# justinhj/minbpe-cc

Hardware: AMD Instinct MI355X
Metric: bpe_train_merges_per_sec (higher is better)
Workload: dtype u16; 1 GPU; BASELINE config 4: SplitMix64(seed 42) uniform-random bytes, 4294967296 bytes whole job, basic encoder (one chunk), vocab 32000, lexicographic tie-break; a step is ONE WHOLE TRAINING (pair-count scan, stream and table setup, every merge up to the vocabulary: 31744 merges); corpus_bytes=4294967296, vocab_size=32000

## Files before the change

### include/mbpe.h

```cpp
#ifndef MBPE_H
#define MBPE_H

#include <stdint.h>

#ifdef __cplusplus
extern "C" {
#endif

#define MBPE_API __attribute__((visibility("default")))

#define MBPE_MAX_VOCAB_BASIC   65534u
#define MBPE_MAX_VOCAB_ENDBIT  32766u
#define MBPE_MAX_VOCAB_CHUNKED 65518u
#define MBPE_MAX_VOCAB_WIDE    16777216u
#define MBPE_NO_BARRIER 0xFFFFFFFFu

typedef enum {
    MBPE_NEED_EXCHANGE =  1,
    MBPE_OK            =  0,
    MBPE_ERR_ARG       = -1,
    MBPE_ERR_NO_DEVICE = -2,
    MBPE_ERR_HIP       = -3,
    MBPE_ERR_VOCAB     = -4,
    MBPE_ERR_STATE     = -5,
    MBPE_ERR_OOM       = -6,
    MBPE_ERR_REGEX     = -7,
    MBPE_ERR_SPLIT_GAP = -8,
    MBPE_ERR_COMM      = -9,
    MBPE_ERR_OVERFLOW  = -10,
    MBPE_ERR_IO        = -11
} mbpe_status;

typedef struct mbpe_ctx mbpe_ctx;

typedef struct {
    uint64_t n_bytes;
    uint64_t n_chunks;
    uint64_t n_slots;
    uint64_t n_live;
    uint32_t n_merges;
    uint32_t n_compactions;
    uint64_t n_pairs;
    float    ms_pair_count;
    float    ms_begin;
    float    ms_steps;
    uint32_t pair_count_launches;
    uint32_t merge_launches;
    float    ms_merge_kernel;
    uint32_t n_batches;
    uint32_t n_fused;
    uint32_t n_fused_dropped;
    uint32_t cut_conflict;
    uint32_t cut_bucket;
    uint32_t cut_single;
    uint32_t cut_full;
    uint32_t n_validation_drops;
    float    ms_grow_table;
    float    ms_compact;
    uint32_t n_table_grows;
    uint32_t n_sel_fallback;
    uint32_t fused_launches;
    float    ms_fused_kernel;
    uint64_t fused_slots;
    uint32_t n_sel_retry;
    uint32_t adapt_limit;
    uint64_t n_sel_blocks;
    uint32_t size_hist[8];
    uint32_t n_skipped;
    uint32_t n_skip_cut;
    uint64_t exchange_words;
    uint32_t exchanges;
    uint32_t pad_;
    uint64_t fused_live_tokens;
    float    ms_pair_count_kernel;
    uint32_t pad2_;
} mbpe_stats;

MBPE_API const char *mbpe_last_error(void);
MBPE_API const char *mbpe_version(void);


MBPE_API int  mbpe_create(int device_id, mbpe_ctx **out);
MBPE_API void mbpe_destroy(mbpe_ctx *ctx);


MBPE_API int mbpe_load_corpus(mbpe_ctx *ctx, const uint8_t *text, uint64_t n_bytes,
                              const uint64_t *chunk_off, uint64_t n_chunks,
                              int text_on_device);

MBPE_API int mbpe_load_corpus_ranges(mbpe_ctx *ctx, const uint8_t *text, uint64_t n_bytes,
                                     const uint64_t *starts, const uint64_t *ends, uint64_t n_chunks,
                                     int text_on_device);

MBPE_API int mbpe_pair_count_u8(mbpe_ctx *ctx, uint32_t *table65536_out);


MBPE_API int mbpe_train_begin(mbpe_ctx *ctx, uint32_t vocab_size);

MBPE_API int mbpe_train_steps(mbpe_ctx *ctx, uint32_t n_steps, uint32_t *steps_done_out);

MBPE_API int mbpe_train_sequences(mbpe_ctx *ctx, uint32_t n_sequences, uint32_t *merges_done_out);

MBPE_API int mbpe_train_result(mbpe_ctx *ctx, uint32_t *merges_out, int32_t *counts_out,
                               uint32_t cap_merges, uint32_t *n_merges_out);

MBPE_API int mbpe_train_lexical(mbpe_ctx *ctx, const uint8_t *text, uint64_t n_bytes,
                                const uint64_t *chunk_off, uint64_t n_chunks,
                                uint32_t vocab_size,
                                uint32_t *merges_out, int32_t *counts_out,
                                uint32_t *n_merges_out, mbpe_stats *stats_out);

MBPE_API int mbpe_train(mbpe_ctx *ctx, const uint8_t *text, uint64_t n_bytes,
                        const uint64_t *chunk_off, uint64_t n_chunks, uint32_t vocab_size,
                        int conflict_resolution,
                        uint32_t *merges_out, int32_t *counts_out,
                        uint32_t *n_merges_out, mbpe_stats *stats_out);

MBPE_API int mbpe_get_stats(mbpe_ctx *ctx, mbpe_stats *out);


MBPE_API int mbpe_get_stream(mbpe_ctx *ctx, uint32_t *tokens_out, uint8_t *chunk_end_out,
                             uint64_t cap, uint64_t *n_out);

MBPE_API int mbpe_stream_device(mbpe_ctx *ctx, const void **slots_out, uint64_t *n_slots_out,
                                uint32_t *slot_bits_out, uint32_t *end_bit_out, uint32_t *barrier_out);

MBPE_API int mbpe_table_device(mbpe_ctx *ctx, const void **cells_out, uint32_t *vshift_out);

MBPE_API int mbpe_get_pairs(mbpe_ctx *ctx, uint32_t *first_out, uint32_t *second_out,
                            int32_t *count_out, uint64_t cap, uint64_t *n_out);

MBPE_API int mbpe_compact(mbpe_ctx *ctx);

MBPE_API int mbpe_set_option(mbpe_ctx *ctx, const char *name, int64_t value);


MBPE_API int mbpe_encode_chunks(int device_id, const uint8_t *text, uint64_t n_bytes,
                                const uint64_t *chunk_off, uint64_t n_chunks,
                                const uint32_t *merges, uint32_t n_merges,
                                uint32_t *tokens_out, uint64_t cap, uint64_t *n_out,
                                uint32_t *n_passes_out);

MBPE_API int mbpe_encode_chunks_device(int device_id, const uint8_t *text, uint64_t n_bytes,
                                       const uint64_t *chunk_off, uint64_t n_chunks,
                                       const uint32_t *merges, uint32_t n_merges,
                                       uint32_t *tokens_dev_out, uint64_t cap, uint64_t *n_out,
                                       uint32_t *n_passes_out);

typedef struct mbpe_encoder mbpe_encoder;
MBPE_API int  mbpe_encoder_create(int device_id, const uint32_t *merges, uint32_t n_merges, mbpe_encoder **out);
MBPE_API void mbpe_encoder_destroy(mbpe_encoder *e);

MBPE_API int  mbpe_encoder_encode(mbpe_encoder *e, const uint8_t *text, uint64_t n_bytes, int text_on_device,
                                  const uint64_t *chunk_off, uint64_t n_chunks,
                                  void *tokens_out, uint64_t cap, uint32_t token_bits, int out_on_device,
                                  uint64_t *chunk_tok_off_out, uint64_t *n_out, uint32_t *n_passes_out);

MBPE_API int  mbpe_encoder_set_option(mbpe_encoder *e, const char *name, int64_t value);
// ... 96 lines not shown
```

### minbpe-cc_amd/csrc/kernels.hip

```cpp
#include "mbpe_dev.h"
#include <hip/hip_ext.h>

#include <cstdlib>

namespace mbpe {

namespace {

constexpr int kWave = 64;
constexpr uint32_t kSent = 0x10000u;

__device__ __forceinline__ uint32_t lane_id() { return threadIdx.x & (kWave - 1); }
__device__ __forceinline__ uint32_t rfl(uint32_t v) { return __builtin_amdgcn_readfirstlane(v); }

typedef unsigned int u32x4 __attribute__((ext_vector_type(4)));

__device__ __forceinline__ uint32_t wave_from_next(uint32_t v, uint32_t edge) {
    return (uint32_t)__builtin_amdgcn_update_dpp((int)edge, (int)v, 0x130, 0xf, 0xf, false);
}
__device__ __forceinline__ uint32_t wave_from_prev(uint32_t v, uint32_t edge) {
    return (uint32_t)__builtin_amdgcn_update_dpp((int)edge, (int)v, 0x138, 0xf, 0xf, false);
}

#define MBPE_GLOBAL_AS __attribute__((address_space(1)))
// ... 1560 lines not shown
}

__global__ void k_apply(PairTable t, DevCtl *ctl, const unsigned long long *__restrict__ best_ptr,
                        uint32_t X, uint32_t *LR, const uint32_t *gm_gadj, TileSum *sums,
                        const TileSum *side, uint32_t *chg, uint32_t n_chg_words, int seq) {
    if (seq) {
        if (ctl->batch_n != 1) return;
        const uint32_t k = ctl->k_done;
        best_ptr += k;
        X = 256u + k;
    }
    const unsigned long long best = *best_ptr;
    const uint32_t x = blockIdx.x * blockDim.x + threadIdx.x;
    if ((best >> 32) != 0) {
        const uint32_t key = ~(uint32_t)best;
        const uint32_t a = key >> 16, b = key & 0xFFFFu;
        patch_sums(sums, side, chg, n_chg_words, x, gridDim.x * blockDim.x);
        const uint32_t pitch = lr_pitch(X);
        for (uint32_t xx = x; xx < X; xx += gridDim.x * blockDim.x) {
            const uint2 lr = make_uint2(LR[lr_idx(pitch, xx, 0, 0)], LR[lr_idx(pitch, xx, 0, 1)]);
            if (lr.x) {
                table_add(t, ctl, (xx << 16) | a, -(int32_t)lr.x, false);
                table_add(t, ctl, (xx << 16) | X, (int32_t)lr.x, true);
            }
            if (lr.y) {
                table_add(t, ctl, (b << 16) | xx, -(int32_t)lr.y, false);
                table_add(t, ctl, (X << 16) | xx, (int32_t)lr.y, true);
            }
            if (lr.x) LR[lr_idx(pitch, xx, 0, 0)] = 0;
            if (lr.y) LR[lr_idx(pitch, xx, 0, 1)] = 0;
        }
        if (x == 0) {
            const uint32_t m = gm_gadj ? gm_gadj[0] : ctl->m;
            const uint32_t adj = gm_gadj ? gm_gadj[1] : ctl->adj;
            if (m) table_add(t, ctl, (a << 16) | b, -(int32_t)m, false);
            if (adj) {
                table_add(t, ctl, (b << 16) | a, -(int32_t)adj, false);
                table_add(t, ctl, (X << 16) | X, (int32_t)adj, true);
            }
            const uint32_t rm = ctl->rm;
            ctl->removed_total += rm;
            ctl->n_live -= rm;
            ctl->m = 0;
            ctl->adj = 0;
            ctl->rm = 0;
        }
    }
}


#ifndef MBPE_PRED_NUM
#define MBPE_PRED_NUM 4
#endif
constexpr uint32_t kBucketKeys = 2;
#ifndef MBPE_LUT_BUCKETS
#define MBPE_LUT_BUCKETS 8192
#endif
constexpr uint32_t kBuckets = MBPE_LUT_BUCKETS;
static_assert((kBuckets & (kBuckets - 1u)) == 0, "the hash is masked");
constexpr uint32_t kEmptyPair = 0xFFFEFFFEu;

static_assert(kBatchMax <= 65536, "batch indices are stored in 16 bits");
constexpr uint32_t kByteCols = 256u + (uint32_t)kTTMax + 1u;
constexpr uint32_t kByteRows = 257u;
struct BatchLutHash {
    uint2 bucket[kBuckets];
    uint32_t bidx[kBuckets];
};
struct BatchLutMem : BatchLutHash {
    uint16_t byte_tail[kByteRows * kByteCols > sizeof(BatchLutHash) / 2 ? kByteRows * kByteCols - sizeof(BatchLutHash) / 2 : 1];
    __device__ __forceinline__ uint16_t *byte_tab() { return reinterpret_cast<uint16_t *>(this); }
};
static_assert(sizeof(BatchLutMem) >= kByteRows * kByteCols * 2, "the byte table overlays the hash table");
#ifndef MBPE_HASH_SEEDS
#define MBPE_HASH_SEEDS 8
#endif
constexpr int kHashSeeds = MBPE_HASH_SEEDS;
__device__ __constant__ const uint32_t kHashMul[8] = {2531u, 40503u, 10007u, 60493u, 25013u, 7919u, 52361u, 33391u};
static_assert(kHashSeeds >= 1 && kHashSeeds <= 8, "kHashMul");
struct BatchLut {
    BatchLutMem *m;
    uint32_t mul;
    bool bytes;
    uint32_t idmask;
    __device__ __forceinline__ BatchLut(BatchLutMem *mem, const BatchState *bs, uint32_t idmask_)
        : m(mem), mul(rfl(bs->hash_mul)), bytes(rfl(bs->byte_lut) != 0u), idmask(idmask_) {}
};

template <bool TT>
__device__ __forceinline__ uint32_t byte_entry(const BatchLut &lut, uint32_t first, uint32_t second, uint32_t idmask) {
    const uint32_t r = first < 256u ? first : 256u;
    uint32_t c = second < 256u ? second : kByteCols - 1u;
    if (TT) {
        const uint32_t i = idmask - 1u - second;
        c = i < (uint32_t)kTTMax ? 256u + i : c;
    }
    return lut.m->byte_tab()[r * kByteCols + c];
}

__device__ __forceinline__ uint32_t pair_hash(uint32_t mul, uint32_t first, uint32_t second) {
    return (__umul24(second, mul) + first) & (kBuckets - 1u);
}
__device__ __forceinline__ uint32_t pair_hash_u(uint32_t uniform_mul, uint32_t first, uint32_t second) {
    uint32_t h;
    asm("v_mad_u32_u24 %0, %1, %2, %3" : "=v"(h) : "v"(second), "s"(uniform_mul), "v"(first));
    return h & (kBuckets - 1u);
}

struct TTInfo {
    uint32_t map[kTTSlots];
    uint32_t tok[kTTMax];
    uint32_t pair[kTTMax];
    uint32_t cnt[kTTMax];
};

__device__ __forceinline__ void tt_build(TTInfo &ti, const BatchState *bs, uint32_t n_keys, uint32_t fake) {
    for (uint32_t i = threadIdx.x; i < kTTSlots; i += blockDim.x) ti.map[i] = 0xFFFFFFFFu;
    for (uint32_t i = threadIdx.x; i < (uint32_t)kTTMax; i += blockDim.x) { ti.tok[i] = kHole; ti.pair[i] = 0; ti.cnt[i] = 0; }
    __syncthreads();
    if (threadIdx.x == 0) {
        uint32_t n = 0;
        for (uint32_t j = 0; j < n_keys && n < (uint32_t)kTTMax; ++j) {
            const uint32_t key = bs->key[j];
            const uint32_t a = key >> 16;
            if ((key & 0xFFFFu) != a) continue;
            ti.map[a & (kTTSlots - 1u)] = a | ((fake - n) << 16);
            ti.tok[n] = a;
            ti.pair[n] = j;
            ++n;
        }
    }
    __syncthreads();
}

__device__ __forceinline__ void tt_flush(TTInfo &ti, uint32_t *hdr_m) {
    __syncthreads();
    if (threadIdx.x < (uint32_t)kTTMax && ti.cnt[threadIdx.x]) atomicAdd(&hdr_m[ti.pair[threadIdx.x]], ti.cnt[threadIdx.x]);
}

constexpr uint32_t kTTMark = 0xFFFEu;
__device__ __forceinline__ void lut_build(BatchLut &lut, const BatchState *bs, uint32_t n_keys, uint32_t fake,
                                          bool tt_marks = false) {
    if (lut.bytes) {
        uint32_t *tw = reinterpret_cast<uint32_t *>(lut.m->byte_tab());
        for (uint32_t i = threadIdx.x; i < (kByteRows * kByteCols + 1u) / 2u; i += blockDim.x) tw[i] = 0xFFFFFFFFu;
        __syncthreads();
        uint16_t *tab = lut.m->byte_tab();
        for (uint32_t j = threadIdx.x; j < n_keys; j += blockDim.x) {
            const uint32_t key = bs->key[j];
            const uint32_t a = key >> 16, b = key & 0xFFFFu;
            if (a != b) tab[a * kByteCols + b] = (uint16_t)j;
        }
        if (threadIdx.x == 0 && bs->tt_index != kNoTT) {
            uint32_t n_tt = 0;
            for (uint32_t j = bs->tt_index; j < n_keys && n_tt < (uint32_t)kTTMax; ++j) {
                const uint32_t key = bs->key[j];
                if ((key >> 16) == (key & 0xFFFFu)) {
                    tab[(key >> 16) * kByteCols + 256u + n_tt++] = (uint16_t)j;
                    if (tt_marks) tab[(key >> 16) * kByteCols + (key >> 16)] = (uint16_t)kTTMark;
                }
            }
        }
        __syncthreads();
        return;
    }
    uint32_t *words = reinterpret_cast<uint32_t *>(lut.m->bucket);
// ... 559 lines not shown
    for (int j = 0; j < 8; ++j) {
        if (s[j] != kHole) {
            if (last == kHole) first_id = s[j] & idmask;
            if ((s[j] & idmask) == last) { ++len; repeats = true; }
            else { full = full && last == kHole; len = 1; }
            lodd |= (len & 1u) ? 0u : 1u << j;
            lead |= full ? 1u << j : 0u;
            last = s[j];
        }
    }
    const bool p1_runs = h.p1 != kHole && !(h.p1 & endbit);
    const uint32_t in_last = h.p1, in_len = p1_runs ? (rb_small & 1u) : 1u;
    uint32_t rl, rn;
    const bool cross = first_id == wave_from_prev(last, in_last);
    if (__ballot(last == kHole) == 0ull && __ballot(repeats || cross) == 0ull) {
        rl = rlane(last, kWave - 1);
        rn = 1u;
    } else {
    auto join = [&](uint32_t o_last, uint32_t o_len, bool o_full) {
        if (last == kHole) { last = o_last; len = o_len; full = o_full; }
        else if (o_last != kHole) {
            if (full && (last & idmask) == o_last) { len += o_len; full = o_full; }
            else full = false;
        }
    };
    if (__ballot(last == kHole || (full && cross)) != 0ull) {
        if (lane == 0) join(in_last, in_len, false);
#pragma unroll
        for (int d = 1; d < kWave; d <<= 1) {
            const uint32_t ol = __shfl_up(last, d, kWave), on = __shfl_up(len | (full ? 0x80000000u : 0u), d, kWave);
            if (lane >= (uint32_t)d) join(ol, on & 0x7FFFFFFFu, (on >> 31) != 0u);
        }
    }
    const uint32_t lv = wave_from_prev(last, in_last), ln = wave_from_prev(len, in_len);
    const uint32_t odd = lodd ^ ((first_id == lv && (ln & 1u)) ? lead : 0u);
    if (__ballot(odd != 0u) != 0ull) {
#pragma unroll
        for (int j = 0; j < 8; ++j)
            if ((odd >> j) & 1u) s[j] = stand_in(s[j]);
    }
    rl = rlane(last, kWave - 1);
    rn = rlane(len, kWave - 1);
    }
    if (h.n1 != kHole) {
        const uint32_t n1 = h.n1;
        const bool c1 = (n1 & idmask) == rl;
        if (c1 && (rn & 1u)) h.n1 = stand_in(n1);
        rn = c1 ? rn + 1u : 1u;
        rl = n1;
        if (h.n2 != kHole && (h.n2 & idmask) == rl && (rn & 1u)) h.n2 = stand_in(h.n2);
    }
    if (p1_runs) {
        const uint32_t p1 = h.p1, p2 = h.p2;
        if (!(rb_small & 1u)) h.p1 = stand_in(p1);
        if (p2 == p1 && (rb_small & 1u)) h.p2 = stand_in(p2);
    }
}

template <int MODE>
__device__ __forceinline__ bool tt_needed(const uint32_t s[8], const uint32_t nxt[8], const Halo &h,
                                          uint32_t tile_first, const TTInfo &ti, uint32_t live_mask = 0xFFu) {
    constexpr uint32_t idmask = MODE == 1 ? 0x7FFFu : 0xFFFFu;
    auto member = [&](uint32_t v) -> bool {
        const uint32_t id = v & idmask;
        return (ti.map[id & (kTTSlots - 1u)] & 0xFFFFu) == id;
    };
    uint32_t eqm = 0;
#pragma unroll
    for (int j = 0; j < 8; ++j) eqm |= (((s[j] ^ nxt[j]) & idmask) == 0u ? 1u : 0u) << j;
    eqm &= live_mask;
    bool need = false;
    if (__ballot(eqm != 0u) != 0ull) {
#pragma unroll
        for (int j = 0; j < 8; ++j)
            if ((eqm >> j) & 1u) need = need || member(s[j]);
    }
    bool hneed = false;
    if (h.p1 != kHole && (((h.p1 ^ tile_first) & idmask) == 0u || (h.p2 != kHole && ((h.p2 ^ h.p1) & idmask) == 0u)))
        hneed = member(h.p1);
    if (h.n1 != kHole && h.n2 != kHole && ((h.n1 ^ h.n2) & idmask) == 0u) hneed = hneed || member(h.n1);
    return __ballot(need) != 0ull || hneed;
}

template <int MODE, int DIAG, bool WRITE, bool TT, class DC>
__device__ __forceinline__ uint4 fused_tile_pf(const uint4 q_orig, const uint32_t s[8], const Halo h,
                                               uint32_t old_x, uint32_t old_y, uint32_t old_z, const BatchLut &lut,
                                               uint32_t X0, uint32_t tile, TileSum *sout, uint32_t *hdr_adj, uint32_t *LR,
                                               DC &dc, bool dc_on, uint32_t &wave_rm, bool &wrote_sum,
                                               __amdgpu_buffer_rsrc_t lr_rsrc, uint32_t adj_pitch, uint16_t *stage,
                                               uint32_t *chg, bool renamed, TTInfo *ti, bool &need_rename,
                                               __amdgpu_buffer_rsrc_t t_rsrc = __amdgpu_buffer_rsrc_t(), bool use_t = false);

template <int MODE, bool HOT, bool TT, int DIAG = 0>
__global__ __launch_bounds__(kLutThreads) void k_scan_batch(const uint16_t *tok0, const uint16_t *tok1,
                                                              const TileSum *__restrict__ sin, uint32_t n_tiles,
                                                              uint32_t *__restrict__ chg, const BatchState *bs,
                                                              uint32_t *hdr_m, uint32_t *hdr_adj, uint32_t *LR,
                                                              const DevCtl *ctl, const RankEdge *le,
                                                              const RankEdge *re,
                                                              const uint32_t *__restrict__ run_in, int hot_launched,
                                                              uint32_t *T) {
    constexpr uint32_t idmask = MODE == 1 ? 0x7FFFu : 0xFFFFu;
    __shared__ BatchLutMem lut_mem;
    const uint32_t waves_per_block = kLutThreads / kWave;
    const uint32_t n_waves = gridDim.x * waves_per_block;
    __shared__ DeltaCache dc;
    const uint32_t n_keys = ctl->batch_n;
    if (n_keys < 2 || ctl->fused) return;
    if ((bs->tt_index != kNoTT) != TT) return;
    __shared__ TTInfo ti;
    const uint16_t *tok = ctl->cur ? tok1 : tok0;
    const uint32_t ctl_k_done = rfl(ctl->k_done);
    const uint32_t adj_pitch = rfl(ctl->adj_pitch);
    if (hot_mismatch<HOT>(bs->packed[0] >> 32, ctl, hot_launched)) return;
    constexpr bool dc_on = HOT;
    if (dc_on) dc_init(dc);
    BatchLut lut(&lut_mem, bs, idmask);
    lut_build(lut, bs, n_keys, idmask - 1u);
    if (TT) tt_build(ti, bs, n_keys, idmask - 1u);
    uint32_t tile = rfl(blockIdx.x * waves_per_block + threadIdx.x / kWave);
    if (tile < n_tiles) {

    const uint32_t last_tile = n_tiles - 1;
    auto clamp_tile = [&](uint64_t t) { return (uint32_t)(t < n_tiles ? t : last_tile); };
    const __amdgpu_buffer_rsrc_t sums_rsrc =
        __builtin_amdgcn_make_buffer_rsrc(const_cast<TileSum *>(sin), 0, n_tiles * 16u, 0x00020000);
    const __amdgpu_buffer_rsrc_t lr_rsrc = __builtin_amdgcn_make_buffer_rsrc(LR, 0, 0xFFFFFFFCu, 0x00020000);
    const bool use_t = T != nullptr && !HOT && ctl->cells_on != 0u && n_keys >= ctl->cells_min;
    const __amdgpu_buffer_rsrc_t t_rsrc = __builtin_amdgcn_make_buffer_rsrc(T ? T : LR, 0, T ? 0xFFFFFFFCu : 0u, 0x00020000);
    TileIn t0 = tile_issue(tok, sums_rsrc, tile);
    TileIn t1 = tile_issue(tok, sums_rsrc, clamp_tile((uint64_t)tile + n_waves));
    bool v1 = (uint64_t)tile + n_waves < n_tiles;
    for (;;) {
        const bool v2 = (uint64_t)tile + 2ull * n_waves < n_tiles;
        TileIn t2 = tile_issue(tok, sums_rsrc, clamp_tile((uint64_t)tile + 2ull * n_waves));

        const uint32_t me_nlive = rlane(t0.smw, 6) & 0xFFFFu;
        if (me_nlive != 0) {
            uint32_t s[8];
            unpack8(t0.q, s);
            Halo h;
            const uint32_t pw1 = rlane(t0.smw, 1), pw2 = rlane(t0.smw, 2);
            const uint32_t nw0 = rlane(t0.smw, 8), nw2 = rlane(t0.smw, 10);
            const bool fast = tile > 0 && tile + 1 < n_tiles && (pw2 & 0xFFFFu) >= 2 && (nw2 & 0xFFFFu) >= 2;
            if (fast) {
                h.p1 = pw1 >> 16; h.p2 = pw1 & 0xFFFFu;
                h.n1 = nw0 & 0xFFFFu; h.n2 = nw0 >> 16;
            } else {
                h = halo_slow(sin, n_tiles, tile, le, re);
            }
            uint32_t rm_unused = 0;
            bool ws_unused = false, no_rename = false;
            if (TT) tt_rename<MODE>(s, h, ti, run_in[tile]);
            fused_tile_pf<MODE, 0, false, TT>(t0.q, s, h, rlane(t0.smw, 4), rlane(t0.smw, 5), rlane(t0.smw, 6), lut,
                                              256u + ctl_k_done, tile, nullptr, hdr_adj, LR, dc, dc_on, rm_unused, ws_unused,
                                              lr_rsrc, adj_pitch, nullptr, chg, TT, &ti, no_rename, t_rsrc, use_t);
        }
        if (!v1) break;
        tile += n_waves;
        t0 = t1; t1 = t2;
        v1 = v2;
    }
    }
    if (dc_on) dc_flush(dc, LR);
    if (TT) {
        tt_flush(ti, hdr_m);
    }
}

template <int MODE, int DIAG, bool WRITE, bool TT, class DC>
__device__ __forceinline__ uint4 fused_tile_pf(const uint4 q_orig, const uint32_t s[8], const Halo h,
                                               uint32_t old_x, uint32_t old_y, uint32_t old_z, const BatchLut &lut,
                                               uint32_t X0, uint32_t tile, TileSum *sout, uint32_t *hdr_adj, uint32_t *LR,
                                               DC &dc, bool dc_on, uint32_t &wave_rm, bool &wrote_sum,
                                               __amdgpu_buffer_rsrc_t lr_rsrc, uint32_t adj_pitch, uint16_t *stage,
                                               uint32_t *chg, bool renamed, TTInfo *ti, bool &need_rename,
                                               __amdgpu_buffer_rsrc_t t_rsrc, bool use_t) {
    constexpr uint32_t idmask = MODE == 1 ? 0x7FFFu : 0xFFFFu;
    constexpr uint32_t endbit = MODE == 1 ? kEndBit : 0u;
    constexpr uint32_t kNone = 0xFFFFu;
    const uint32_t pitch = lr_pitch(X0);
    const uint32_t xcd_off = DIAG == 6 ? (__builtin_amdgcn_s_getreg((3 << 11) | 20) & 7u) * (2u * 512u * pitch) : 0u;
    auto delta_add = [&](uint32_t idx, uint32_t delta) {
        if (dc_on) dc_add(dc, true, LR, idx, delta);
        else __builtin_amdgcn_raw_ptr_buffer_atomic_add_i32((int)delta, lr_rsrc, (idx + xcd_off) << 2, 0, 0);
    };
    uint32_t lane = lane_id();
    asm volatile("" : "+v"(lane));
    const uint32_t live = old_z & 0xFFFFu;
    if (live == 0u) return q_orig;
    uint32_t tile_first = old_x & 0xFFFFu, tile_last = old_y >> 16;
    if (TT && renamed) {
        const uint32_t li = live - 1u;
        uint32_t sl = s[0];
#pragma unroll
        for (uint32_t j = 1; j < 8; ++j) sl = (li & 7u) == j ? s[j] : sl;
        tile_first = rlane(s[0], 0);
        tile_last = rlane(sl, li >> 3);
    }
    uint32_t n[8];
#pragma unroll
    for (int j = 0; j < 7; ++j) n[j] = s[j + 1];
    n[7] = wave_from_next(s[0], h.n1);
    const uint32_t ef = lane == 0 ? h.p1 : lane == 1 ? h.p2 : lane == 2 ? tile_last : (TT && lane == 3) ? h.n1 : kHole;
    const uint32_t es = (lane == 0 ? tile_first : lane == 1 ? h.p1 : (TT && lane == 3) ? h.n2 : h.n1) & idmask;
    uint32_t idx[8], eidx;
    if (lut.bytes) {
#pragma unroll
        for (int j = 0; j < 8; ++j) idx[j] = byte_entry<TT>(lut, s[j], MODE == 1 ? n[j] & idmask : n[j], idmask);
        eidx = byte_entry<TT>(lut, ef, es, idmask);
        const uint32_t all = idx[0] & idx[1] & idx[2] & idx[3] & idx[4] & idx[5] & idx[6] & idx[7] & eidx;
        if (__ballot(all != kNone) == 0ull && DIAG != 3 && DIAG != 5) return q_orig;
        if (TT) {
            bool mark = eidx == kTTMark;
#pragma unroll
            for (int j = 0; j < 8; ++j) mark = mark || idx[j] == kTTMark;
            if (__ballot(mark) != 0ull) {
                if (!renamed) { need_rename = true; return q_orig; }
#pragma unroll
                for (int j = 0; j < 8; ++j) idx[j] = idx[j] == kTTMark ? kNone : idx[j];
                eidx = eidx == kTTMark ? kNone : eidx;
            }
            eidx = lane == 3 ? kNone : eidx;
        }
    } else {
        uint32_t Hm = 0, Wm = 0;
        {
            bool second_key;
            const bool hit = pair_hit2(lut, ef, es, second_key) && !(TT && lane == 3);
            Hm = hit ? 1u : 0u;
            Wm = second_key ? 1u : 0u;
        }
#pragma unroll
        for (int j = 7; j >= 0; --j) {
            bool second_key;
            const bool hit = pair_hit2(lut, s[j], MODE == 1 ? n[j] & idmask : n[j], second_key);
            Hm = Hm + Hm + (hit ? 1u : 0u);
            Wm = Wm + Wm + (second_key ? 1u : 0u);
        }
        if (__ballot(Hm != 0u) == 0ull && DIAG != 3 && DIAG != 5) return q_orig;
#pragma unroll
        for (int j = 0; j < 8; ++j) {
            idx[j] = kNone;
            if (__ballot(((Hm >> j) & 1u) != 0u) != 0ull) {
                const uint32_t got = lut_index_known(lut, s[j], MODE == 1 ? n[j] & idmask : n[j], ((Wm >> j) & 1u) != 0u);
                idx[j] = (Hm >> j) & 1u ? got : kNone;
            }
        }
        eidx = kNone;
        if (__ballot(((Hm >> 8) & 1u) != 0u) != 0ull) {
            const uint32_t got = lut_index_known(lut, ef, es, ((Wm >> 8) & 1u) != 0u);
            eidx = (Hm >> 8) & 1u ? got : kNone;
        }
    }
    if (DIAG == 3 || DIAG == 5) {
#pragma unroll
        for (int j = 0; j < 8; ++j) asm volatile("" :: "v"(idx[j]));
        asm volatile("" :: "v"(eidx));
        return q_orig;
    }
    const uint32_t in1 = rlane(eidx, 0), in2 = rlane(eidx, 1), out1 = rlane(eidx, 2);
    {
        const uint32_t li = live - 1u;
        const bool mine = lane == (li >> 3);
#pragma unroll
        for (uint32_t j = 0; j < 8; ++j)
            if ((li & 7u) == j) { n[j] = mine ? h.n1 : n[j]; idx[j] = mine ? out1 : idx[j]; }
    }
    const uint32_t prev7 = wave_from_prev(idx[7] | (s[7] << 16), in1 | (h.p1 << 16));
    const uint32_t prev6 = wave_from_prev(idx[6], in2);
    const int lrem = (int)live - (int)(lane * 8u);
    const uint32_t Lm = lrem >= 8 ? 0xFFu : lrem <= 0 ? 0u : (1u << lrem) - 1u;
    uint32_t Am = 0, Bm = 0;
#pragma unroll
    for (int j = 0; j < 8; ++j) {
        const uint32_t pj = j == 0 ? (prev7 & 0xFFFFu) : idx[j - 1];
        Am |= (idx[j] != kNone ? 1u : 0u) << j;
        Bm |= (pj != kNone ? 1u : 0u) << j;
    }
    Bm &= Lm;
    const uint32_t ABm = Am | Bm;
    if (__ballot(ABm != 0u) == 0ull) return q_orig;

    uint32_t n2_7 = wave_from_next(n[0], h.n2);
    uint32_t n2_patch = kSent;
    if (out1 != kNone) {
        const uint32_t li = live - 1u;
        if (lane == (li >> 3)) n2_patch = li & 7u;
    }
    uint32_t out[8];
#pragma unroll
    for (int j = 0; j < 8; ++j) {
        const uint32_t self = s[j];
        uint32_t nv = ((Bm >> j) & 1u) ? kHole : self;
        if (__ballot(((Am >> j) & 1u) != 0u) != 0ull) {
            if ((Am >> j) & 1u) {
                const uint32_t p1 = j == 0 ? prev7 >> 16 : s[j > 0 ? j - 1 : 0];
                const uint32_t ppj = j == 0 ? prev6 : j == 1 ? (prev7 & 0xFFFFu) : idx[j > 1 ? j - 2 : 0];
                const uint32_t ja = idx[j];
                const uint32_t btok = n[j];
                uint32_t n2 = j < 7 ? n[j < 7 ? j + 1 : 7] : n2_7;
                n2 = n2_patch == (uint32_t)j ? h.n2 : n2;
                nv = (X0 + ja) | (btok & endbit);
                if (TT && renamed && (btok & idmask) >= idmask - (uint32_t)kTTMax)
                    atomicAdd(&ti->cnt[idmask - 1u - (btok & idmask)], 1u);
                if (DIAG != 2) {
                    const bool lo = left_open<MODE>(p1), ro = right_open<MODE>(btok, n2);
                    const uint32_t xl = p1 & idmask, yr = n2 & idmask;
                    if (use_t && lo && ro && ppj == kNone && xl < 256u && yr < 256u) {
                        __builtin_amdgcn_raw_ptr_buffer_atomic_add_i32(1, t_rsrc, ((ja << 16) | (xl << 8) | yr) << 2, 0, 0);
                    } else {
                        if (lo) {
                            if (ppj != kNone) {
                                atomicAdd(&hdr_adj[ppj * adj_pitch + ja], 1u);
                                delta_add(lr_idx(pitch, self, ppj, 1), 0xFFFFFFFFu);
                            } else {
                                delta_add(lr_idx(pitch, xl, ja, 0u), 1u);
                            }
                        }
                        if (ro) delta_add(lr_idx(pitch, yr, ja, 1u), 1u);
                    }
                }
            }
        }
        out[j] = nv;
    }
    if (TT && renamed) {
#pragma unroll
        for (int j = 0; j < 8; ++j)
            if (out[j] != kHole && (out[j] & idmask) >= idmask - (uint32_t)kTTMax)
                out[j] = ti->tok[idmask - 1u - (out[j] & idmask)] | (out[j] & endbit);
    }
    if (!WRITE) {
        if (lane == 0) atomicOr(&chg[tile >> 5], 1u << (tile & 31u));
        return q_orig;
    }
    uint32_t n_out;
    const uint4 qc = tile_compact(out, stage, n_out);
    wave_rm += live - n_out;
    uint32_t em = lane == 0 ? 3u : 0u;
    {
        const uint32_t l1 = live - 1u, l2 = live >= 2u ? live - 2u : 0u;
        em |= lane == (l1 >> 3) ? 1u << (l1 & 7u) : 0u;
        em |= lane == (l2 >> 3) ? 1u << (l2 & 7u) : 0u;
    }
    const bool edge = __ballot((ABm & em) != 0u) != 0ull;
    uint4 ns;
    if (edge || (old_z >> 16) != 1u) {
        uint32_t c[8];
        unpack8(qc, c);
        ns = wave_summary(c);
    } else {
        ns = make_uint4(old_x, old_y, (old_z & 0xFFFF0000u) | n_out, 0u);
    }
    if (lane == 0) reinterpret_cast<uint4 *>(sout)[tile] = ns;
    wrote_sum = true;
    return qc;
}

#ifndef MBPE_SKIP_PENALTY0
#define MBPE_SKIP_PENALTY0 2
#endif
#ifndef MBPE_SKIP_PENALTY_MAX
#define MBPE_SKIP_PENALTY_MAX 256
#endif
#ifndef MBPE_FUSED_WAVES
#define MBPE_FUSED_WAVES 4
#endif
template <int MODE, bool HOT, bool TT, int DIAG = 0>
__global__ __launch_bounds__(kLutThreads, MBPE_FUSED_WAVES * 256 / kLutThreads) void k_fused_batch(uint16_t *tok0, uint16_t *tok1,
                                                               const TileSum *__restrict__ sin,
                                                               TileSum *__restrict__ sout, uint32_t n_tiles,
                                                               uint32_t *__restrict__ chg, const BatchState *bs,
                                                               uint32_t *hdr_adj, uint32_t *LR, DevCtl *ctl,
                                                               const RankEdge *le, const RankEdge *re,
                                                               uint32_t *hdr_m, const uint32_t *__restrict__ run_in,
                                                               int hot_launched, uint32_t *T) {
    constexpr uint32_t idmask = MODE == 1 ? 0x7FFFu : 0xFFFFu;
    __shared__ BatchLutMem lut_mem;
    const uint32_t lane = lane_id();
    const uint32_t waves_per_block = kLutThreads / kWave;
    const uint32_t n_waves = gridDim.x * waves_per_block;
    __shared__ DeltaCacheSmall dc;
    const uint32_t n_keys = ctl->batch_n;
    if (n_keys < 2 || !ctl->fused) return;
    if ((bs->tt_index != kNoTT) != TT) return;
    __shared__ TTInfo ti;
    __shared__ __attribute__((aligned(16))) uint16_t stage_mem[kLutThreads / kWave][kTileSlots];
    uint16_t *stage = stage_mem[threadIdx.x / kWave];
    const uint16_t *tok = ctl->cur ? tok1 : tok0;
    uint16_t *dst = ctl->cur ? tok0 : tok1;
    const uint32_t X0 = 256u + ctl->k_done;
    if (hot_mismatch<HOT>(bs->packed[0] >> 32, ctl, hot_launched)) return;
    constexpr bool dc_on = HOT;
    if (dc_on) dc_init(dc);
    BatchLut lut(&lut_mem, bs, idmask);
    lut_build(lut, bs, n_keys, idmask - 1u, TT);
    if (TT) tt_build(ti, bs, n_keys, idmask - 1u);
    if (blockIdx.x == 0 && threadIdx.x == 0) ctl->marks_all = 1;
    uint32_t tile = rfl(blockIdx.x * waves_per_block + threadIdx.x / kWave);
    uint32_t wave_rm = 0;
    if (tile < n_tiles) {

    const uint32_t last_tile = n_tiles - 1;
    auto clamp_tile = [&](uint64_t t) { return (uint32_t)(t < n_tiles ? t : last_tile); };
    const __amdgpu_buffer_rsrc_t sums_rsrc =
        __builtin_amdgcn_make_buffer_rsrc(const_cast<TileSum *>(sin), 0, n_tiles * 16u, 0x00020000);
    const __amdgpu_buffer_rsrc_t lr_rsrc = __builtin_amdgcn_make_buffer_rsrc(LR, 0, 0xFFFFFFFCu, 0x00020000);
    const bool use_t = T != nullptr && !HOT && ctl->cells_on != 0u && n_keys >= ctl->cells_min;
    const __amdgpu_buffer_rsrc_t t_rsrc = __builtin_amdgcn_make_buffer_rsrc(T ? T : LR, 0, T ? 0xFFFFFFFCu : 0u, 0x00020000);
    const uint32_t adj_pitch = rfl(ctl->adj_pitch);
#ifndef MBPE_FUSED_DEPTH
#define MBPE_FUSED_DEPTH 2
#endif
    constexpr int kDepth = MBPE_FUSED_DEPTH;
    TileIn ring[kDepth];
#pragma unroll
    for (int d = 0; d < kDepth; ++d) ring[d] = tile_issue(tok, sums_rsrc, clamp_tile((uint64_t)tile + (uint64_t)d * n_waves));
    for (;;) {
        const bool v1 = (uint64_t)tile + n_waves < n_tiles;
        const TileIn t_new = tile_issue(tok, sums_rsrc, clamp_tile((uint64_t)tile + (uint64_t)kDepth * n_waves));
        const TileIn t0 = ring[0];

        uint4 outq = t0.q;
        bool wrote_sum = false;
        const uint32_t old_x = rlane(t0.smw, 4), old_y = rlane(t0.smw, 5), old_z = rlane(t0.smw, 6);
        if (DIAG == 4) {
            asm volatile("" :: "v"(t0.smw));
        } else if ((old_z & 0xFFFFu) != 0) {
            uint32_t s[8];
            unpack8(t0.q, s);
            Halo h;
            const uint32_t pw1 = rlane(t0.smw, 1), pw2 = rlane(t0.smw, 2);
            const uint32_t nw0 = rlane(t0.smw, 8), nw2 = rlane(t0.smw, 10);
            const bool fast = tile > 0 && tile + 1 < n_tiles && (pw2 & 0xFFFFu) >= 2 && (nw2 & 0xFFFFu) >= 2;
            if (fast) {
                h.p1 = pw1 >> 16; h.p2 = pw1 & 0xFFFFu;
                h.n1 = nw0 & 0xFFFFu; h.n2 = nw0 >> 16;
            } else {
                h = halo_slow(sin, n_tiles, tile, le, re);
            }
            bool renamed = false;
            bool need_rename = false;
            if (TT && !lut.bytes) {
                uint32_t nx[8];
#pragma unroll
                for (int j = 0; j < 7; ++j) nx[j] = s[j + 1];
                nx[7] = wave_from_next(s[0], h.n1);
                const uint32_t li = (old_z & 0xFFFFu) - 1u;
                const bool mine = lane == (li >> 3);
#pragma unroll
                for (uint32_t j = 0; j < 8; ++j)
                    if ((li & 7u) == j) nx[j] = mine ? h.n1 : nx[j];
                const int lrem = (int)(old_z & 0xFFFFu) - (int)(lane * 8u);
                const uint32_t lm = lrem >= 8 ? 0xFFu : lrem <= 0 ? 0u : (1u << lrem) - 1u;
                if (tt_needed<MODE>(s, nx, h, old_x & 0xFFFFu, ti, lm)) {
                    tt_rename<MODE>(s, h, ti, run_in[tile]);
                    renamed = true;
                }
            }
            outq = fused_tile_pf<MODE, DIAG, true, TT>(t0.q, s, h, old_x, old_y, old_z, lut, X0, tile, sout, hdr_adj, LR, dc,
                                                       dc_on, wave_rm, wrote_sum, lr_rsrc, adj_pitch, stage, chg, renamed, &ti,
                                                       need_rename, t_rsrc, use_t);
            if (TT && need_rename) {
                tt_rename<MODE>(s, h, ti, run_in[tile]);
                outq = fused_tile_pf<MODE, DIAG, true, TT>(t0.q, s, h, old_x, old_y, old_z, lut, X0, tile, sout, hdr_adj, LR,
                                                           dc, dc_on, wave_rm, wrote_sum, lr_rsrc, adj_pitch, stage, chg, true,
                                                           &ti, need_rename, t_rsrc, use_t);
            }
        }
        if (!wrote_sum && lane == 0) reinterpret_cast<uint4 *>(sout)[tile] = make_uint4(old_x, old_y, old_z, 0u);
        MBPE_GLOBAL_AS char *obase =
            (MBPE_GLOBAL_AS char *)uniform_ptr(reinterpret_cast<uintptr_t>(dst) + (uint64_t)tile * (kWave * 16u));
        u32x4 oq; oq.x = outq.x; oq.y = outq.y; oq.z = outq.z; oq.w = outq.w;
        __builtin_nontemporal_store(oq, (MBPE_GLOBAL_AS u32x4 *)(obase + lane * 16u));

        if (!v1) break;
        tile += n_waves;
#pragma unroll
        for (int d = 0; d + 1 < kDepth; ++d) ring[d] = ring[d + 1];
        ring[kDepth - 1] = t_new;
    }
    }
    if (dc_on) dc_flush(dc, LR);
    if (lane == 0 && wave_rm) atomicAdd(&ctl->rm, wave_rm);
    if (TT) {
        tt_flush(ti, hdr_m);
    }
}

__global__ __launch_bounds__(256) void k_pair_cells_fold(uint32_t *__restrict__ T, uint32_t *__restrict__ LR, const DevCtl *ctl) {
    __shared__ uint32_t rows[256];
    const uint32_t n = ctl->batch_n;
    if (n < ctl->cells_min || !ctl->cells_on) return;
    const uint32_t pitch = lr_pitch(256u + ctl->k_done);
    uint32_t hits = 0;
    const uint32_t t = threadIdx.x;
    for (uint32_t j = blockIdx.x; j < n; j += gridDim.x) {
        uint32_t *tj = T + (size_t)j * 65536u;
        rows[t] = 0;
        __syncthreads();
        uint32_t col = 0;
#pragma unroll 8
        for (uint32_t x = 0; x < 256u; ++x) {
            const uint32_t v = tj[x * 256u + t];
            if (__ballot(v != 0u) == 0ull) continue;
            if (v) tj[x * 256u + t] = 0;
            col += v;
            const uint32_t rs = wave_sum(v);
            if (lane_id() == 0 && rs) atomicAdd(&rows[x], rs);
        }
        __syncthreads();
        if (col) LR[lr_idx(pitch, t, j, 1u)] += col;
        if (rows[t]) LR[lr_idx(pitch, t, j, 0u)] += rows[t];
        hits += col;
        __syncthreads();
    }
    hits = wave_sum(hits);
    if (lane_id() == 0 && hits) atomicAdd(const_cast<uint32_t *>(&ctl->cell_hits), hits);
}


__global__ __launch_bounds__(kWave) void k_adj_sums(const uint32_t *__restrict__ hdr_adj, BatchState *bs, const DevCtl *ctl) {
    const uint32_t n = ctl->batch_n;
    if (n < 2) return;
    for (uint32_t j = blockIdx.x; j < n; j += gridDim.x) {
        uint32_t in = 0, out = 0;
        for (uint32_t p = threadIdx.x; p < n; p += kWave) { in += hdr_adj[p * ctl->adj_pitch + j]; out += hdr_adj[j * ctl->adj_pitch + p]; }
        in = wave_sum(in);
        out = wave_sum(out);
        if (threadIdx.x == 0) { bs->adj_in[j] = in; bs->adj_out[j] = out; }
    }
}

constexpr uint32_t kLrChunk = 4096;
__global__ __launch_bounds__(256) void k_delta_max(const uint32_t *__restrict__ LR, BatchState *bs, const DevCtl *ctl) {
    const uint32_t n_keys = ctl->batch_n;
    if (n_keys < 2) return;
    const uint32_t X = 256u + ctl->k_done;
    const uint32_t pitch = lr_pitch(X);
    const uint32_t chunks = (X + kLrChunk - 1u) / kLrChunk;
    const uint32_t n_items = 2u * n_keys * chunks;
    for (uint32_t item = blockIdx.x; item < n_items; item += gridDim.x) {
        const uint32_t row = item / chunks, x0 = (item - row * chunks) * kLrChunk;
        const uint32_t j = row >> 1, side = row & 1u, Xj = X + j;
        const uint32_t add = side ? bs->adj_out[j] : bs->adj_in[j];
        const uint32_t *cells = LR + (size_t)row * pitch;
        unsigned long long mp = 0;
#pragma unroll 4
        for (uint32_t x = x0 + threadIdx.x; x < x0 + kLrChunk && x < X; x += 256u) {
            const uint32_t v = cells[x];
            if (v) {
                const unsigned long long p = pack_best((int32_t)(v + add), side ? (Xj << 16) | x : (x << 16) | Xj);
                mp = p > mp ? p : mp;
            }
        }
        mp = wave_max_u64(mp);
        if (lane_id() == 0 && mp > __hip_atomic_load(&bs->maxp[j], __ATOMIC_RELAXED, __HIP_MEMORY_SCOPE_AGENT))
            atomicMax(&bs->maxp[j], mp);
    }
}

constexpr int kValThreads = kBatchMax < 256 ? 256 : kBatchMax > 1024 ? 1024 : kBatchMax;
constexpr int kValSlots = kBatchMax < 256 ? 256 : kBatchMax;
__global__ __launch_bounds__(256) void k_adj_max(const uint32_t *__restrict__ hdr_adj, BatchState *bs, const DevCtl *ctl) {
    const uint32_t n = ctl->batch_n;
    if (n < 2) return;
    const uint32_t X0 = 256u + ctl->k_done;
    const uint32_t n_waves = gridDim.x * (blockDim.x / kWave);
    for (uint32_t p = blockIdx.x * (blockDim.x / kWave) + threadIdx.x / kWave; p < n; p += n_waves) {
        for (uint32_t q = lane_id(); q < n; q += kWave) {
// ... 330 lines not shown
}

__global__ void k_list_marked(const uint32_t *__restrict__ chg, uint32_t n_words, uint32_t *__restrict__ list,
                              DevCtl *ctl, uint32_t n_tiles) {
    if (ctl->batch_n < 2 || (ctl->fused && ctl->commit_n == ctl->batch_n)) return;
    const uint32_t w = blockIdx.x * blockDim.x + threadIdx.x;
    uint32_t bits = w < n_words ? chg[w] : 0u;
    if (ctl->marks_all && w < n_words) {
        const uint32_t left = n_tiles - w * 32u;
        bits = left >= 32u ? 0xFFFFFFFFu : (1u << left) - 1u;
    }
    const uint32_t cnt = __popc(bits);
    const uint32_t incl = wave_incl_scan(cnt);
    const uint32_t total = __shfl(incl, kWave - 1, kWave);
    uint32_t base = 0;
    if (lane_id() == 0 && total) base = atomicAdd(&ctl->n_marked, total);
    base = __shfl(base, 0, kWave) + incl - cnt;
    while (bits) {
        list[base++] = w * 32u + (uint32_t)__builtin_ctz(bits);
        bits &= bits - 1;
    }
}

template <int MODE, bool TT>
__global__ __launch_bounds__(kLutThreads) void k_rewrite_marked(uint16_t *tok0, uint16_t *tok1,
                                                                  const TileSum *__restrict__ sin,
                                                                  TileSum *__restrict__ sout, uint32_t n_tiles,
                                                                  uint32_t *__restrict__ chg,
                                                                  const uint32_t *__restrict__ list,
                                                                  const BatchState *bs, DevCtl *ctl,
                                                                  const RankEdge *le, const RankEdge *re,
                                                                  const uint32_t *__restrict__ run_in) {
    constexpr uint32_t idmask = MODE == 1 ? 0x7FFFu : 0xFFFFu;
    __shared__ BatchLutMem lut_mem;
    if (ctl->batch_n < 2 || (ctl->fused && ctl->commit_n == ctl->batch_n)) return;
    uint16_t *tok = ctl->cur ? tok1 : tok0;
    const uint32_t n_keys = ctl->commit_n;
    if ((bs->tt_index < n_keys) != TT) return;
    __shared__ TTInfo ti;
    __shared__ __attribute__((aligned(16))) uint16_t stage_mem[kLutThreads / kWave][kTileSlots];
    uint16_t *stage = stage_mem[threadIdx.x / kWave];
    const uint32_t X0 = 256u + ctl->k_done;
    const uint32_t n_list = ctl->n_marked;
    const bool marks_all = ctl->marks_all != 0u;
    BatchLut lut(&lut_mem, bs, idmask);
    lut_build(lut, bs, n_keys, idmask - 1u);
    if (TT) tt_build(ti, bs, n_keys, idmask - 1u);
    const uint32_t lane = lane_id();
    const uint32_t waves_per_block = kLutThreads / kWave;
    const uint32_t n_waves = gridDim.x * waves_per_block;
    uint32_t i = rfl(blockIdx.x * waves_per_block + threadIdx.x / kWave);
    if (i >= n_list) return;
    const __amdgpu_buffer_rsrc_t sums_rsrc =
        __builtin_amdgcn_make_buffer_rsrc(const_cast<TileSum *>(sin), 0, n_tiles * 16u, 0x00020000);
    const uint32_t last = n_list - 1;
    auto tile_at = [&](uint64_t k) { return list[k < n_list ? k : last]; };
    uint32_t tile0 = tile_at(i), tile1 = tile_at((uint64_t)i + n_waves), tile2 = tile_at((uint64_t)i + 2ull * n_waves);
    TileIn t0 = tile_issue(tok, sums_rsrc, tile0);
    TileIn t1 = tile_issue(tok, sums_rsrc, tile1);
    uint32_t wave_rm = 0;
    for (;;) {
        const bool has_next = (uint64_t)i + n_waves < n_list;
        const uint32_t tile3 = tile_at((uint64_t)i + 3ull * n_waves);
        const TileIn t2 = tile_issue(tok, sums_rsrc, tile2);

        const uint32_t tile = tile0;
        uint32_t s[8];
        unpack8(t0.q, s);
        Halo h;
        const uint32_t pw1 = rlane(t0.smw, 1), pw2 = rlane(t0.smw, 2);
        const uint32_t nw0 = rlane(t0.smw, 8), nw2 = rlane(t0.smw, 10);
        const bool fast = tile > 0 && tile + 1 < n_tiles && (pw2 & 0xFFFFu) >= 2 && (nw2 & 0xFFFFu) >= 2;
        if (fast) {
            h.p1 = pw1 >> 16; h.p2 = pw1 & 0xFFFFu;
            h.n1 = nw0 & 0xFFFFu; h.n2 = nw0 >> 16;
        } else {
            h = halo_slow(sin, n_tiles, tile, le, re);
        }
        uint32_t rm = 0;
        bool wrote = false;
        bool no_rename = false;
        DeltaCacheSmall no_dc;
        if (TT) tt_rename<MODE>(s, h, ti, run_in[tile]);
        const uint4 qn = fused_tile_pf<MODE, 2, true, TT>(t0.q, s, h, rlane(t0.smw, 4), rlane(t0.smw, 5), rlane(t0.smw, 6), lut,
                                                          X0, tile, sout, nullptr, nullptr, no_dc, false, rm, wrote,
                                                          __amdgpu_buffer_rsrc_t(), 0u, stage, chg, TT, &ti, no_rename);
        if (wrote) {
            reinterpret_cast<uint4 *>(tok)[(uint64_t)tile * kWave + lane] = qn;
            if (lane == 0 && marks_all) atomicOr(&chg[tile >> 5], 1u << (tile & 31u));
        } else if (lane == 0 && !marks_all) {
            atomicAnd(&chg[tile >> 5], ~(1u << (tile & 31u)));
        }
        wave_rm += rm;

        if (!has_next) break;
        i += n_waves;
        tile0 = tile1; tile1 = tile2; tile2 = tile3;
        t0 = t1; t1 = t2;
    }
    if (lane == 0 && wave_rm) atomicAdd(&ctl->rm, wave_rm);
}

__global__ void k_seq_finish(DevCtl *ctl, uint32_t *fused_flag, const BatchState *bs) {
    if (blockIdx.x || threadIdx.x) return;
    const uint32_t bs_skip_n = bs->skip_n;
    const uint32_t rm_seq = ctl->batch_n >= 2 ? ctl->rm : 0u;
    if (fused_flag) *fused_flag = ctl->fused && ctl->batch_n >= 2 ? 1u : 0u;
    if (ctl->batch_n >= 2) {
        const uint32_t rm = ctl->rm;
        ctl->removed_total += rm;
        ctl->n_live -= rm;
        ctl->rm = 0;
    }
    if (ctl->batch_n >= 2) {
        uint32_t lim = ctl->adapt_limit ? ctl->adapt_limit : (uint32_t)kBatchMax;
        if (ctl->commit_n < ctl->batch_n) lim = ctl->commit_n * 2u < 4u ? 4u : ctl->commit_n * 2u;
        else if (ctl->batch_n >= lim) lim = lim * 2u;
        ctl->adapt_limit = lim > (uint32_t)kBatchMax ? (uint32_t)kBatchMax : lim;
    }
    if (ctl->skip_off) ctl->skip_off -= 1;
    if (ctl->batch_n >= 2 && ctl->skip_failed) {
        const uint32_t pen = ctl->skip_penalty ? (ctl->skip_penalty * 2u > (uint32_t)MBPE_SKIP_PENALTY_MAX ? (uint32_t)MBPE_SKIP_PENALTY_MAX : ctl->skip_penalty * 2u)
                                               : (uint32_t)MBPE_SKIP_PENALTY0;
        ctl->skip_penalty = pen;
        ctl->skip_off = pen;
    } else if (ctl->batch_n >= 2 && bs_skip_n > 0 && ctl->skip_penalty) {
        ctl->skip_penalty /= 2u;
    }
    ctl->skip_failed = 0;
    if (ctl->cells_on && ctl->cells_min >= kCellsMinBatch && ctl->batch_n >= ctl->cells_min &&
        ctl->cell_hits * 2ull < (unsigned long long)rm_seq)
        ctl->cells_on = 0;
    ctl->cell_hits = 0;
    if (ctl->fused && ctl->batch_n >= 2) {
        ctl->n_fused += 1;
        if (ctl->commit_n == ctl->batch_n) ctl->cur ^= 1u;
        else ctl->n_fused_dropped += 1;
    }
    ctl->fused = 0;
    ctl->marks_all = 0;
    if (ctl->commit_n) ctl->size_hist[31 - __builtin_clz(ctl->commit_n) > 7 ? 7 : 31 - __builtin_clz(ctl->commit_n)] += 1;
    if (fused_flag) {
        fused_flag[1] = (uint32_t)ctl->n_live;
        fused_flag[2] = (uint32_t)(ctl->n_live >> 32);
        fused_flag[3] = ctl->commit_n;
    }
    ctl->k_done += ctl->commit_n;
    ctl->batch_n = 0;
    ctl->commit_n = 0;
    ctl->n_marked = 0;
}


constexpr int kScanThreads = 256;
constexpr int kScanPerThread = 16;
constexpr uint32_t kScanChunk = kScanThreads * kScanPerThread;

__device__ __forceinline__ unsigned long long block_sum_u64(unsigned long long v, unsigned long long *sh) {
#pragma unroll
    for (int d = kWave / 2; d > 0; d >>= 1) v += shfl_xor_u64(v, d);
    __syncthreads();
    if (lane_id() == 0) sh[threadIdx.x / kWave] = v;
    __syncthreads();
    unsigned long long r = 0;
    for (uint32_t w = 0; w < blockDim.x / kWave; ++w) r += sh[w];
    return r;
}

__global__ __launch_bounds__(kScanThreads) void k_tile_scan_partial(const TileSum *__restrict__ sums,
                                                                    uint32_t n_tiles,
                                                                    unsigned long long *__restrict__ part) {
    __shared__ unsigned long long sh[kScanThreads / kWave];
    const uint64_t base = (uint64_t)blockIdx.x * kScanChunk;
    unsigned long long s = 0;
    for (uint32_t i = threadIdx.x; i < kScanChunk; i += kScanThreads)
        if (base + i < n_tiles) s += sums[base + i].n_live;
    s = block_sum_u64(s, sh);
    if (threadIdx.x == 0) part[blockIdx.x] = s;
}

__global__ __launch_bounds__(1024) void k_tile_scan_top(unsigned long long *__restrict__ part, uint32_t n_parts,
                                                        DevCtl *ctl) {
    __shared__ unsigned long long tot[1024];
    const uint32_t per = (n_parts + 1023u) / 1024u;
    const uint32_t lo = threadIdx.x * per < n_parts ? threadIdx.x * per : n_parts;
    const uint32_t hi = lo + per < n_parts ? lo + per : n_parts;
    unsigned long long s = 0;
    for (uint32_t i = lo; i < hi; ++i) s += part[i];
    tot[threadIdx.x] = s;
    __syncthreads();
    if (threadIdx.x == 0) {
        unsigned long long run = 0;
        for (int i = 0; i < 1024; ++i) { const unsigned long long v = tot[i]; tot[i] = run; run += v; }
        ctl->scan_total = run;
    }
    __syncthreads();
    unsigned long long run = tot[threadIdx.x];
    for (uint32_t i = lo; i < hi; ++i) { const unsigned long long v = part[i]; part[i] = run; run += v; }
}

__global__ __launch_bounds__(kScanThreads) void k_tile_scan_final(const TileSum *__restrict__ sums, uint32_t n_tiles,
                                                                  const unsigned long long *__restrict__ part,
                                                                  unsigned long long *__restrict__ offsets) {
    __shared__ unsigned long long th[kScanThreads];
    const uint64_t first = (uint64_t)blockIdx.x * kScanChunk + (uint64_t)threadIdx.x * kScanPerThread;
    uint32_t v[kScanPerThread];
    unsigned long long s = 0;
#pragma unroll
    for (int i = 0; i < kScanPerThread; ++i) {
        v[i] = first + i < n_tiles ? sums[first + i].n_live : 0u;
        s += v[i];
    }
    th[threadIdx.x] = s;
    __syncthreads();
    if (threadIdx.x == 0) {
        unsigned long long run = part[blockIdx.x];
// ... 304 lines not shown
    if (!v.n_tiles) return;
    const uint32_t n_chunks = (v.n_tiles + kRunChunk - 1) / kRunChunk;
    hipLaunchKernelGGL(k_run_partial, dim3(n_chunks), dim3(kRunThreads), 0, v.stream, v.sums, v.n_tiles, best, v.ctl, seq, bs,
                       v.run_part);
    hipLaunchKernelGGL(k_run_final, dim3(n_chunks), dim3(kRunThreads), 0, v.stream, v.sums, v.n_tiles, best, v.ctl, seq, bs,
                       v.run_part, v.left_edge, v.run_in);
}

void launch_merge(const StreamView &v, const BatchView &b, const unsigned long long *best, uint32_t new_id,
                  uint32_t *m_adj, int seq, const Inst &w) {
    if (!v.n_tiles) return;
    const BatchState *bs = seq ? b.bs : nullptr;
    if (inst_may_tt(w)) launch_run_lengths(v, bs, best, seq);
    static const int occ[3] = {resident_blocks(k_merge<0, false, 0>), resident_blocks(k_merge<1, false, 0>),
                               resident_blocks(k_merge<2, false, 0>)};
    const dim3 grid(tile_grid(v.n_tiles, v.n_cus, occ[slot_mode(v.endbit)])), block(kMergeThreads);
    const int hot_launched = w.hot;
#define MBPE_MERGE_ARGS v.tok, v.tok_other, v.sums, v.side, v.n_tiles, v.chg, best, new_id, b.LR, v.ctl, m_adj, v.left_edge, \
                        v.right_edge, seq, v.run_in, hot_launched
#ifdef MBPE_DIAG
    static const int diag = getenv("MBPE_MERGE_DIAG") ? atoi(getenv("MBPE_MERGE_DIAG")) : 0;
    if (diag == 1 && !v.endbit) {
        hipLaunchKernelGGL((k_merge<0, false, 1>), grid, block, 0, v.stream, MBPE_MERGE_ARGS);
        return;
    }
    if (diag == 2 && !v.endbit) {
        hipLaunchKernelGGL((k_merge<0, false, 2>), grid, block, 0, v.stream, MBPE_MERGE_ARGS);
        return;
    }
#endif
    MBPE_BY_MODE(v.endbit, {
        if (inst_takes(w, w.tt, false)) hipLaunchKernelGGL((k_merge<M, false, 0>), grid, block, 0, v.stream, MBPE_MERGE_ARGS);
        if (inst_takes(w, w.tt, true)) hipLaunchKernelGGL((k_merge<M, true, 0>), grid, block, 0, v.stream, MBPE_MERGE_ARGS);
    });
#undef MBPE_MERGE_ARGS
}

void launch_apply(const StreamView &v, const BatchView &b, PairTable t, const unsigned long long *best, uint32_t new_id,
                  const uint32_t *gm_gadj, int seq) {
    const uint32_t n_words = (v.n_tiles + 31u) / 32u;
    uint32_t blocks = (new_id + 255) / 256;
    const uint32_t want = (n_words + 255) / 256;
    if (want > blocks) blocks = want < 2048 ? want : 2048;
    hipLaunchKernelGGL(k_apply, dim3(blocks), dim3(256), 0, v.stream, t, v.ctl, best, new_id, b.LR, gm_gadj, v.sums, v.side,
                       v.chg, n_words, seq);
}

void launch_patch_sums(const StreamView &v, const unsigned long long *best, int seq) {
    const uint32_t n_words = (v.n_tiles + 31u) / 32u;
    uint32_t blocks = (n_words + 255) / 256;
    if (blocks > 2048) blocks = 2048;
    if (blocks < 1) blocks = 1;
    hipLaunchKernelGGL(k_patch_sums, dim3(blocks), dim3(256), 0, v.stream, best, v.sums, v.side, v.chg, n_words, v.ctl, seq,
                       v.n_tiles);
}

void launch_select_batch(const StreamView &v, const BatchView &b, PairTable t, unsigned long long *best,
                         const SelectArgs &a, int attempts, int first_attempt, bool fallback) {
    const hipStream_t s = v.stream;
    const uint32_t fake_id = (v.endbit == kEndBit ? 0x7FFFu : 0xFFFFu) - 1u;
    const uint32_t tt_max = 256u + a.n_target <= fake_id + 1u - (uint32_t)kTTMax ? (uint32_t)kTTMax : 1u;
    const uint32_t sel_cap = a.sel_cap < 64u ? 64u : a.sel_cap > kSelCap ? kSelCap : a.sel_cap;
    if (a.sel) {
        const int blocks = (v.n_cus > 0 ? v.n_cus : 256) * 4;
        for (int attempt = first_attempt < 0 ? 0 : first_attempt; attempt < (attempts < 1 ? 1 : attempts > 3 ? 3 : attempts); ++attempt) {
            hipLaunchKernelGGL(k_sel_scan, dim3(blocks), dim3(256), 0, s, t, v.ctl, a.sel, a.n_target, sel_cap, attempt);
            hipLaunchKernelGGL(k_sel_pick, dim3(1), dim3(kPickThreads), 0, s, v.ctl, b.bs, a.sel, best, a.n_target, a.max_batch,
                               a.fused_min, (uint32_t)v.n_ranks, attempt, fake_id, sel_cap, tt_max, a.byte_table ? 1u : 0u);
        }
    }
    if (fallback)
        hipLaunchKernelGGL(k_select_batch, dim3(1), dim3(kHierThreads), 0, s, t, v.ctl, b.bs, best, a.n_target, a.max_batch,
                           a.fused_min, (uint32_t)v.n_ranks);
}

void launch_fused_batch(const StreamView &v, const BatchView &b, const Inst &w) {
    if (!v.n_tiles) return;
    static const int occ[3] = {resident_blocks(k_fused_batch<0, false, false, 0>, kLutThreads),
                               resident_blocks(k_fused_batch<1, false, false, 0>, kLutThreads),
                               resident_blocks(k_fused_batch<2, false, false, 0>, kLutThreads)};
    const dim3 grid(tile_grid(v.n_tiles, v.n_cus, occ[slot_mode(v.endbit)], kLutThreads)), block(kLutThreads);
    const int hot_launched = w.hot;
#define MBPE_FUSED_ARGS v.tok, v.tok_other, v.sums, v.side, v.n_tiles, v.chg, b.bs, b.hdr_adj, b.LR, v.ctl, v.left_edge, \
                        v.right_edge, b.hdr_m, v.run_in, hot_launched, b.pair_cells
#ifdef MBPE_DIAG
    const int diag = getenv("MBPE_FUSED_DIAG") ? atoi(getenv("MBPE_FUSED_DIAG")) : 0;
#define MBPE_FUSED_DIAG_CASE(D)                                                                                            \
    if (diag == D && !v.endbit) {                                                                                          \
        hipLaunchKernelGGL((k_fused_batch<0, false, false, D>), grid, block, 0, v.stream, MBPE_FUSED_ARGS);                \
        hipLaunchKernelGGL((k_fused_batch<0, false, true, D>), grid, block, 0, v.stream, MBPE_FUSED_ARGS);                 \
        return;                                                                                                            \
    }
    MBPE_FUSED_DIAG_CASE(2)
    MBPE_FUSED_DIAG_CASE(3)
    MBPE_FUSED_DIAG_CASE(4)
    MBPE_FUSED_DIAG_CASE(5)
    MBPE_FUSED_DIAG_CASE(6)
#undef MBPE_FUSED_DIAG_CASE
#endif
    MBPE_BY_MODE(v.endbit, MBPE_BY_INST(w, hipLaunchKernelGGL((k_fused_batch<M, HOT, TT>), grid, block, 0, v.stream, MBPE_FUSED_ARGS)));
#undef MBPE_FUSED_ARGS
}

void launch_scan_batch(const StreamView &v, const BatchView &b, const Inst &w) {
    if (!v.n_tiles) return;
    static const int occ[3] = {resident_blocks(k_scan_batch<0, false, false, 0>, kLutThreads),
                               resident_blocks(k_scan_batch<1, false, false, 0>, kLutThreads),
                               resident_blocks(k_scan_batch<2, false, false, 0>, kLutThreads)};
    const dim3 grid(tile_grid(v.n_tiles, v.n_cus, occ[slot_mode(v.endbit)], kLutThreads)), block(kLutThreads);
    const int hot_launched = w.hot;
    MBPE_BY_MODE(v.endbit, MBPE_BY_INST(w, hipLaunchKernelGGL((k_scan_batch<M, HOT, TT, 0>), grid, block, 0, v.stream, v.tok,
                                                             v.tok_other, v.sums, v.n_tiles, v.chg, b.bs, b.hdr_m, b.hdr_adj, b.LR,
                                                             v.ctl, v.left_edge, v.right_edge, v.run_in, hot_launched,
                                                             b.pair_cells)));
}

void launch_pair_cells_fold(const StreamView &v, const BatchView &b, uint32_t n_hint) {
    if (!b.pair_cells) return;
    if (n_hint < 64u) n_hint = 64u;
    if (n_hint > 1024u) n_hint = 1024u;
    hipLaunchKernelGGL(k_pair_cells_fold, dim3(n_hint), dim3(256), 0, v.stream, b.pair_cells, b.LR, v.ctl);
}

void launch_batch_tables(const StreamView &v, const BatchView &b, PairTable t, uint32_t id_upper, uint32_t n_hint) {
    const hipStream_t s = v.stream;
    if (n_hint < 64u) n_hint = 64u;
    if (n_hint > (uint32_t)kBatchMax) n_hint = kBatchMax;
    const uint64_t cells = (uint64_t)id_upper * kBatchMax;
    uint32_t blocks = (uint32_t)((cells + 255) / 256);
    if (blocks > 2048) blocks = 2048;
    if (blocks < 8) blocks = 8;
    hipLaunchKernelGGL(k_adj_sums, dim3(n_hint), dim3(kWave), 0, s, b.hdr_adj, b.bs, v.ctl);
    hipLaunchKernelGGL(k_delta_max, dim3(blocks < 1024 ? blocks : 1024), dim3(256), 0, s, b.LR, b.bs, v.ctl);
    hipLaunchKernelGGL(k_adj_max, dim3(n_hint / 4), dim3(256), 0, s, b.hdr_adj, b.bs, v.ctl);
    hipLaunchKernelGGL(k_validate, dim3(1), dim3(kValThreads), 0, s, t, v.ctl, b.bs, b.hdr_m, b.hdr_adj, b.LR);
    if (t.cells) {
        uint32_t j_parts = (n_hint + kApplyTile - 1) / kApplyTile;
        if (j_parts > kApplyJParts) j_parts = kApplyJParts;
        uint32_t grid = ((id_upper + kApplyTile - 1) / kApplyTile) * j_parts;
        if (grid < 256u) grid = 256u;
        hipLaunchKernelGGL(k_apply_batch_dense, dim3(grid), dim3(256), 0, s, t, v.ctl, b.bs, b.hdr_m, b.hdr_adj, b.LR, j_parts);
    } else {
        hipLaunchKernelGGL(k_apply_batch, dim3(blocks), dim3(256), 0, s, t, v.ctl, b.bs, b.hdr_m, b.hdr_adj, b.LR);
    }
}

void launch_rewrite_marked(const StreamView &v, const BatchView &b, const Inst &w) {
    if (!v.n_tiles) return;
    const uint32_t n_words = (v.n_tiles + 31u) / 32u;
    hipLaunchKernelGGL(k_list_marked, dim3((n_words + 255) / 256), dim3(256), 0, v.stream, v.chg, n_words, v.tile_list, v.ctl,
                       v.n_tiles);
    static const int occ[3] = {resident_blocks(k_rewrite_marked<0, false>, kLutThreads),
                               resident_blocks(k_rewrite_marked<1, false>, kLutThreads),
                               resident_blocks(k_rewrite_marked<2, false>, kLutThreads)};
    const dim3 grid(tile_grid(v.n_tiles, v.n_cus, occ[slot_mode(v.endbit)], kLutThreads)), block(kLutThreads);
#define MBPE_REWRITE_ARGS v.tok, v.tok_other, v.sums, v.side, v.n_tiles, v.chg, v.tile_list, b.bs, v.ctl, v.left_edge, \
                          v.right_edge, v.run_in
    MBPE_BY_MODE(v.endbit, {
        hipLaunchKernelGGL((k_rewrite_marked<M, false>), grid, block, 0, v.stream, MBPE_REWRITE_ARGS);
        if (inst_may_tt(w)) hipLaunchKernelGGL((k_rewrite_marked<M, true>), grid, block, 0, v.stream, MBPE_REWRITE_ARGS);
    });
#undef MBPE_REWRITE_ARGS
}

__global__ void k_seq_info(const DevCtl *ctl, const BatchState *bs, const unsigned long long *best, uint32_t *out) {
    if (blockIdx.x || threadIdx.x) return;
    const uint32_t n = ctl->batch_n;
    unsigned long long top = 0;
    uint32_t tt = 0;
    if (n >= 2) {
        top = bs->packed[0] >> 32;
        tt = bs->tt_index != kNoTT ? 1u : 0u;
    } else if (n == 1) {
        const unsigned long long b = best[ctl->k_done];
        const uint32_t key = ~(uint32_t)b;
        top = b >> 32;
        tt = (top != 0 && (key >> 16) == (key & 0xFFFFu)) ? 1u : 0u;
    }
    out[0] = ctl->k_done;
    out[1] = n;
    out[2] = ctl->fused;
    out[3] = tt;
    out[4] = dc_wanted(top, ctl->n_live * ctl->n_ranks) ? 1u : 0u;
    out[5] = ctl->k_limit;
    out[6] = ctl->sel_ok;
    out[7] = 0;
}

void launch_seq_info(const StreamView &v, const BatchView &b, const unsigned long long *best, uint32_t *out) {
    hipLaunchKernelGGL(k_seq_info, dim3(1), dim3(64), 0, v.stream, v.ctl, b.bs, best, out);
}

void launch_seq_finish(const StreamView &v, const BatchView &b, uint32_t *fused_flag) {
    hipLaunchKernelGGL(k_seq_finish, dim3(1), dim3(64), 0, v.stream, v.ctl, fused_flag, b.bs);
}

void launch_tile_scan(const StreamView &v, unsigned long long *offsets) {
    if (!v.n_tiles) return;
    unsigned long long *part = offsets + v.n_tiles;
    const uint32_t n_parts = (v.n_tiles + kScanChunk - 1) / kScanChunk;
    hipLaunchKernelGGL(k_tile_scan_partial, dim3(n_parts), dim3(kScanThreads), 0, v.stream, v.sums, v.n_tiles, part);
    hipLaunchKernelGGL(k_tile_scan_top, dim3(1), dim3(1024), 0, v.stream, part, n_parts, v.ctl);
    hipLaunchKernelGGL(k_tile_scan_final, dim3(n_parts), dim3(kScanThreads), 0, v.stream, v.sums, v.n_tiles, part, offsets);
}

void launch_compact_scatter(const StreamView &v, const unsigned long long *offsets) {
    if (!v.n_tiles) return;
    hipLaunchKernelGGL(k_compact_scatter, dim3(tile_grid(v.n_tiles, v.n_cus)), dim3(kMergeThreads), 0, v.stream, v.tok, v.sums,
                       offsets, v.n_tiles, v.tok_other);
}

void launch_rank_edge(const StreamView &v, uint32_t *hdr) {
    hipLaunchKernelGGL(k_rank_edge, dim3(1), dim3(64), 0, v.stream, v.sums, v.n_tiles, reinterpret_cast<RankEdge *>(hdr + 2) + v.rank,
                       v.ctl, hdr);
}

void launch_compose_edges(hipStream_t s, uint32_t *hdr, int rank, int n_ranks, RankEdge *left, RankEdge *right) {
    hipLaunchKernelGGL(k_compose_edges, dim3(1), dim3(64), 0, s, hdr, rank, n_ranks, left, right);
}

void launch_boundary_pairs(hipStream_t s, uint32_t *bp, const uint32_t *hdr, int n_ranks, uint32_t endbit, uint32_t *pcount) {
    hipLaunchKernelGGL(k_boundary_pairs, dim3(1), dim3(64), 0, s, bp, hdr, n_ranks, endbit, pcount);
}

void launch_pair_total(hipStream_t s, const uint32_t *bp, const uint32_t *pcount, unsigned long long expect,
                       unsigned long long *sum_out, DevCtl *ctl) {
    hipLaunchKernelGGL(k_pair_total, dim3(1), dim3(1024), 0, s, bp, pcount, expect, sum_out, ctl);
}

}
```

### minbpe-cc_amd/csrc/mbpe_dev.h

```cpp
#ifndef MBPE_DEV_H
#define MBPE_DEV_H

#include <hip/hip_runtime.h>
#include <stdint.h>

namespace mbpe {

constexpr uint32_t kHole = 0xFFFFu;
constexpr uint32_t kEndBit = 0x8000u;
constexpr uint32_t kBarrier = 0xFFEEu;

constexpr int kTile = 512;
constexpr int kMergeThreads = 256;
#ifndef MBPE_LUT_THREADS
#define MBPE_LUT_THREADS 1024
#endif
constexpr int kLutThreads = MBPE_LUT_THREADS;
constexpr int kSlotsPerLane = 8;

struct __attribute__((aligned(16))) TileSum {
    uint16_t head0, head1;
    uint16_t tail1, tail0;
    uint16_t n_live;
    uint16_t tail_run;
    uint16_t pad0, pad1;
};
static_assert(sizeof(TileSum) == 16, "TileSum must be 16 bytes");

struct RankEdge {
    uint32_t head0, head1;
    uint32_t tail1, tail0;
    uint32_t n_live_lo, n_live_hi;
    uint32_t tail_run_lo, tail_run_hi;
};

constexpr uint32_t kEmptyKey = 0xFFFFFFFFu;
constexpr unsigned long long kEmptySlot = 0xFFFFFFFFFFFFFFFFull;

constexpr int kBlockShift = 10;
constexpr uint32_t kBlockSize = 1u << kBlockShift;

struct PairTable {
    unsigned long long *hslot;
    uint32_t *ekey;
    int32_t  *ecnt;
    unsigned long long *bmax;
    unsigned long long *smax;
    uint32_t  hmask;
    uint32_t  ecap;
    uint32_t *cells;
    uint32_t  vshift;
};
constexpr uint32_t kPresent = 0x80000000u;

struct DevCtl {
    uint32_t n_entries;
    uint32_t err;
    uint32_t m;
    uint32_t adj;
    unsigned long long removed_total;
    unsigned long long n_live;
    unsigned long long scan_total;
    uint32_t rm;
    uint32_t k_done;
    uint32_t k_limit;
    uint32_t batch_n;
    uint32_t commit_n;
    uint32_t n_batches;
    uint32_t n_marked;
    uint32_t cur;
    uint32_t fused;
    uint32_t n_fused;
    uint32_t n_fused_dropped;
    uint32_t cut_conflict, cut_bucket, cut_single, cut_full;
    uint32_t n_validation_drops;
    unsigned long long sel_T;
    uint32_t sel_n;
    uint32_t sel_ok;
    uint32_t n_sel_fallback;
    uint32_t sel_retry;
    uint32_t adapt_limit;
    uint32_t recent_n;
    uint32_t n_sel_retry;
    uint32_t sel_mode;
    uint32_t n_ranks;
    uint32_t size_hist[8];
    uint32_t n_skipped;
    uint32_t n_skip_cut;
    uint32_t skip_off;
    uint32_t skip_penalty;
    uint32_t skip_failed;
    uint32_t skip_red_q16;
    unsigned long long n_sel_blocks;
    uint32_t first_mode;
    uint32_t first_tie;
    uint32_t marks_all;
    uint32_t cells_on;
    uint32_t cell_hits;
    uint32_t cells_min;
    uint32_t adj_pitch;

};

#ifndef MBPE_BATCH_MAX
#define MBPE_BATCH_MAX 4096
#endif
constexpr int kBatchMax = MBPE_BATCH_MAX;
constexpr int kBatchDefault = kBatchMax;
static_assert((kBatchMax & (kBatchMax - 1)) == 0 && kBatchMax >= 64,
              "a power of two: grid strides over the delta arrays keep a thread on one pair index");
#ifndef MBPE_SEL_CAP
#define MBPE_SEL_CAP 8192
#endif
constexpr uint32_t kSelCap = MBPE_SEL_CAP;
struct SelList {
    unsigned long long packed[kSelCap];
    uint32_t eidx[kSelCap];
};

#ifndef MBPE_TT_MAX
#define MBPE_TT_MAX 16
#endif
constexpr int kTTMax = MBPE_TT_MAX;
static_assert(0xFFFFu - (uint32_t)MBPE_TT_MAX > kBarrier, "the barrier id must lie below the stand-in ids");
constexpr uint32_t kTTSlots = 256;
#ifndef MBPE_SKIP_MAX
#define MBPE_SKIP_MAX 32
#endif
constexpr int kSkipMax = MBPE_SKIP_MAX;
constexpr uint32_t kCellsMinBatch = 512;
constexpr uint32_t kNoTT = 0xFFFFFFFFu;
struct BatchState {
    uint32_t key[kBatchMax];
    uint32_t eidx[kBatchMax];
    unsigned long long packed[kBatchMax];
    unsigned long long maxp[kBatchMax];
    uint32_t adj_in[kBatchMax];
    uint32_t adj_out[kBatchMax];
    uint32_t tt_index;
    uint32_t tt_token;
    uint32_t tt_n;
    uint32_t hash_mul;
    uint32_t byte_lut;
    uint32_t skip_n;
    uint32_t skip_key[kSkipMax];
    uint32_t skip_pos[kSkipMax];
    unsigned long long skip_packed[kSkipMax];
};

inline uint32_t batch_header_words(uint32_t adj_pitch) { return (uint32_t)kBatchMax + adj_pitch * adj_pitch; }
__host__ __device__ inline uint32_t lr_pitch(uint32_t ids) { return (ids + 63u) & ~63u; }
__host__ __device__ inline unsigned long long lr_words(uint32_t ids, uint32_t n_pairs) {
    return 2ull * (n_pairs ? n_pairs : 1u) * lr_pitch(ids);
}

constexpr uint32_t kErrTableFull   = 1u;
constexpr uint32_t kErrNegCount    = 2u;
constexpr uint32_t kErrMissingPair = 4u;
constexpr uint32_t kErrCountRange  = 8u;
constexpr uint32_t kErrHotSkipped  = 16u;

__host__ __device__ inline unsigned long long pack_best(int32_t count, uint32_t key) {
    return ((unsigned long long)(uint32_t)count << 32) | (uint32_t)(~key);
}

struct StreamView {
    hipStream_t stream;
    uint16_t *tok, *tok_other;
    TileSum *sums;
    TileSum *side;
    uint32_t n_tiles;
    uint32_t *chg;
    uint32_t *tile_list;
    uint32_t *run_in;
    unsigned long long *run_part;
    DevCtl *ctl;
    const RankEdge *left_edge, *right_edge;
    int rank, n_ranks;
    uint32_t endbit;
    int n_cus;
};

struct BatchView {
    BatchState *bs;
    uint32_t *hdr_m, *hdr_adj;
    uint32_t *LR;
    uint32_t *pair_cells;
};

struct Inst { bool known, tt, hot; };
inline Inst inst_any(bool hot_possible) { return Inst{false, false, hot_possible}; }
inline Inst inst_known(bool tt, bool hot) { return Inst{true, tt, hot}; }
inline bool inst_takes(const Inst &w, bool tt, bool hot) { return w.known ? w.tt == tt && w.hot == hot : !hot || w.hot; }
inline bool inst_may_tt(const Inst &w) { return !w.known || w.tt; }

void launch_fill_u32(hipStream_t s, uint32_t *p, uint64_t n, uint32_t v);
void launch_fill_u16(hipStream_t s, uint16_t *p, uint64_t n, uint16_t v);

size_t pair_count_scratch_bytes(int n_workgroups);
void launch_pair_count_u8(hipStream_t s, const uint8_t *text, uint64_t n,
                          const uint8_t *endmask, uint32_t *bp, int n_workgroups, uint32_t *scratch,
                          hipEvent_t start = nullptr, hipEvent_t stop = nullptr);

void launch_widen(hipStream_t s, const uint8_t *text, uint64_t n, const uint8_t *endmask,
                  uint16_t *tok, uint64_t n_slots_padded);
void launch_widen_barrier(hipStream_t s, const uint8_t *text, uint64_t n, const uint8_t *endmask,
                          uint16_t *tok, uint64_t n_slots);

void launch_summarize(const StreamView &v);

void launch_table_init(hipStream_t s, const uint32_t *bp, PairTable t, DevCtl *ctl);
void launch_table_rehash(hipStream_t s, PairTable t, DevCtl *ctl);

void launch_argmax(hipStream_t s, PairTable t, const DevCtl *ctl, unsigned long long *best, bool hierarchical);

size_t first_state_bytes();
void launch_first_init(hipStream_t s, void *fs);
void launch_first_tiebreak(const StreamView &v, PairTable t, unsigned long long *best, void *fs, uint32_t *xf, int seq,
                           int phase);

void launch_merge(const StreamView &v, const BatchView &b, const unsigned long long *best, uint32_t new_id,
                  uint32_t *m_adj, int seq, const Inst &w);
void launch_run_lengths(const StreamView &v, const BatchState *bs, const unsigned long long *best, int seq);

void launch_apply(const StreamView &v, const BatchView &b, PairTable t, const unsigned long long *best, uint32_t new_id,
                  const uint32_t *gm_gadj, int seq);
void launch_patch_sums(const StreamView &v, const unsigned long long *best, int seq);

struct SelectArgs {
    SelList *sel;
    uint32_t n_target, max_batch, fused_min, sel_cap;
    bool byte_table;
};
void launch_select_batch(const StreamView &v, const BatchView &b, PairTable t, unsigned long long *best,
                         const SelectArgs &a, int attempts = 3,
                         int first_attempt = 0 ,
                         bool fallback = true );
void launch_scan_batch(const StreamView &v, const BatchView &b, const Inst &w);
void launch_fused_batch(const StreamView &v, const BatchView &b, const Inst &w);
void launch_pair_cells_fold(const StreamView &v, const BatchView &b, uint32_t n_hint);
void launch_batch_tables(const StreamView &v, const BatchView &b, PairTable t, uint32_t id_upper, uint32_t n_hint);
void launch_rewrite_marked(const StreamView &v, const BatchView &b, const Inst &w);
void launch_seq_info(const StreamView &v, const BatchView &b, const unsigned long long *best, uint32_t *out);
void launch_seq_finish(const StreamView &v, const BatchView &b, uint32_t *fused_flag);

inline size_t tile_scan_scratch(uint32_t n_tiles) { return (size_t)n_tiles / 4096 + 2; }
void launch_tile_scan(const StreamView &v, unsigned long long *offsets);
void launch_compact_scatter(const StreamView &v, const unsigned long long *offsets);

inline uint32_t exchange_header_words(int n_ranks) { return (uint32_t)((2 + 8 * n_ranks + 3) / 4 * 4); }
void launch_rank_edge(const StreamView &v, uint32_t *hdr);
void launch_compose_edges(hipStream_t s, uint32_t *hdr, int rank, int n_ranks, RankEdge *left, RankEdge *right);
constexpr uint32_t kPairCountWords = 4;
void launch_boundary_pairs(hipStream_t s, uint32_t *bp, const uint32_t *hdr, int n_ranks, uint32_t endbit,
                           uint32_t *pcount);
void launch_pair_total(hipStream_t s, const uint32_t *bp, const uint32_t *pcount, unsigned long long expect,
// ... 6 lines not shown
```

### minbpe-cc_amd/csrc/train.cpp

```cpp
#include "mbpe.h"
#include "mbpe_dev.h"
#include "wide.h"
#include "hip_host.h"

#include <dlfcn.h>
#include <rccl/rccl.h>

#include <algorithm>
#include <chrono>
#include <cstddef>
#include <cstdio>
#include <cstring>
#include <map>
#include <string>
#include <unordered_map>
#include <vector>

using namespace mbpe;

namespace {

#define HIPCHK(expr) MBPE_HIP_CHECK(expr, false)

uint64_t round_up(uint64_t v, uint64_t m) { return (v + m - 1) / m * m; }
// ... 7 lines not shown
bool stoi_parses(const uint8_t *s, uint64_t n) { long long v; return stoi_value(s, n, &v); }

template <typename T>
void dfree(T *&p) {
    if (p) { (void)hipFree(p); p = nullptr; }
}

}

struct mbpe_ctx;
namespace {
template <typename T> hipError_t tmalloc(mbpe_ctx *c, T **p, size_t bytes);
template <typename T> void tfree(mbpe_ctx *c, T *&p);
void pool_trim(mbpe_ctx *c);
}

namespace {
struct Rccl {
    void *lib = nullptr;
    int (*GetUniqueId)(void *) = nullptr;
    int (*CommInitRank)(void **, int, ncclUniqueId, int) = nullptr;
    int (*CommDestroy)(void *) = nullptr;
    int (*AllReduce)(const void *, void *, size_t, int, int, void *, hipStream_t) = nullptr;
    const char *(*GetErrorString)(int) = nullptr;
    bool ok = false;
    std::string why;
};

Rccl &rccl() {
    static Rccl r;
    static bool tried = false;
    if (tried) return r;
    tried = true;
    for (const char *n : {"librccl.so.1", "librccl.so", "/opt/rocm/lib/librccl.so.1"}) {
        r.lib = dlopen(n, RTLD_NOW | RTLD_LOCAL);
        if (r.lib) break;
    }
    if (!r.lib) { r.why = "librccl.so.1 not found"; return r; }
#define MBPE_BIND(field, name) \
    r.field = reinterpret_cast<decltype(r.field)>(dlsym(r.lib, name)); \
    if (!r.field) { r.why = std::string("missing RCCL symbol ") + name; return r; }
    MBPE_BIND(GetUniqueId, "ncclGetUniqueId")
    MBPE_BIND(CommInitRank, "ncclCommInitRank")
    MBPE_BIND(CommDestroy, "ncclCommDestroy")
    MBPE_BIND(AllReduce, "ncclAllReduce")
    MBPE_BIND(GetErrorString, "ncclGetErrorString")
#undef MBPE_BIND
    r.ok = true;
    return r;
}
}

struct mbpe_ctx {
    int device = 0;
    hipStream_t stream = nullptr;
    hipEvent_t ev0 = nullptr, ev1 = nullptr;
    int n_cus = 256;

    const uint8_t *d_text = nullptr;
    uint8_t *d_text_owned = nullptr;
    uint8_t *d_endmask = nullptr;
    uint64_t n_bytes = 0;
    uint64_t n_chunks = 0;
    bool chunked = false;
    uint64_t n_barriers = 0;
    bool barrier = false;
    bool loaded = false;
    bool inert = false;

    uint32_t *pc_scratch = nullptr;
    uint32_t *pc_bp = nullptr;
    void *first_state = nullptr;
    uint32_t *xf = nullptr;

    uint16_t *tok[2] = {nullptr, nullptr};
    int cur = 0;
    uint64_t cap_slots = 0;
    uint64_t n_slots = 0;
    uint32_t n_tiles = 0;
    TileSum *sums = nullptr;
    TileSum *side = nullptr;
    uint32_t *chg = nullptr;
    uint32_t *tile_list = nullptr;
    SelList *sel = nullptr;
    uint32_t *run_in = nullptr;
    int seq_slot = -1;
    unsigned long long *offsets = nullptr;

    PairTable tab = {};
    uint32_t hcap = 0;
    DevCtl *ctl = nullptr;
    unsigned long long *best = nullptr;
    uint32_t *xb = nullptr;
    uint32_t hdr_words = 0;
    uint32_t hdrb_words = 0;
    uint32_t *hdr_m = nullptr, *hdr_adj = nullptr;
    uint32_t *LR = nullptr;
    BatchState *bs = nullptr;
    uint32_t *xb0 = nullptr;
    uint32_t h_pcount[kPairCountWords] = {};
    uint32_t *pair_cells = nullptr;
    RankEdge *d_left = nullptr, *d_right = nullptr;

    uint32_t vocab_size = 0;
    uint32_t n_target = 0;
    uint32_t k = 0;
    uint32_t n_valid = 0;
    bool begun = false;
    bool exhausted = false;
    double merges_per_seq = 0;
    uint32_t first_b = 0, first_s = 0;
    bool first_legacy = false;
    DevCtl h_ctl = {};

    int rank = 0, n_ranks = 1;
    bool comm_external = false;
    void *nccl_comm = nullptr;
    int pending = 0;
    uint32_t pending_target = 0;

    int64_t opt_compact_den = 16;
    int64_t opt_batch = 16;
    int64_t opt_time_kernels = 0;
    int64_t opt_force_exchange = 0;
    int64_t opt_hier_argmax = -1;
    int64_t opt_multi_merge = 1;
    int64_t opt_max_batch = kBatchDefault;
    int64_t opt_fused_min = 24;
    bool opt_byte_table = true;
    int64_t opt_sel_cap = kSelCap;
    int64_t opt_threshold_select = 1;
    int64_t opt_dense_table = -1;
    int hot_possible = 1;
    unsigned long long last_top = ~0ull;
    int64_t opt_barrier = -1;
    int64_t opt_first_batches = 0;
    int64_t opt_first = 0;
    int64_t opt_pc_repeat = 1;
    uint32_t k_upper = 0;
    int sel_attempts = 3;
    uint32_t max_batch_eff = kBatchMax, adj_pitch = kBatchMax;
    uint32_t *h_seq = nullptr;
    uint32_t *d_seq_info = nullptr;
    int64_t opt_pair_cells = -1;
    int64_t opt_lockstep = -1;
    hipEvent_t ev_sel = nullptr;
    std::vector<hipEvent_t> kev;
    std::vector<hipEvent_t> kev_f;
    uint32_t *seq_flags = nullptr;
    std::vector<uint32_t> h_seq_flags;

    bool wide = false;
    bool wide_active = false;
    uint32_t vocab_total = 0;
    uint32_t n_target_total = 0;
    int64_t opt_wide_from = -1;
    int64_t opt_first_wide = 0;
    bool wfirst = false;
    uint32_t *wtok[2] = {nullptr, nullptr};
    int wcur = 0;
    uint32_t *wval = nullptr, *wscratch = nullptr;
    WideTable wtab = {};
    WideCtl *wctl = nullptr;
    WideBest *wbest = nullptr;
    unsigned long long *warg = nullptr;
    WideFirst *wfs = nullptr;
    uint64_t wn_upper = 0;
    uint32_t wk = 0;
    WideCtl h_wctl = {};
    std::vector<WideBest> h_wbest;

    mbpe_stats stats = {};

    std::unordered_map<void *, size_t> pool_live;
    std::multimap<size_t, void *> pool_idle;
};

namespace {

template <typename T>
hipError_t tmalloc(mbpe_ctx *c, T **p, size_t bytes) {
    if (bytes == 0) bytes = 4;
    auto it = c->pool_idle.find(bytes);
    if (it != c->pool_idle.end()) {
        *p = static_cast<T *>(it->second);
        c->pool_live[it->second] = bytes;
        c->pool_idle.erase(it);
        return hipSuccess;
    }
    void *q = nullptr;
    hipError_t e = hipMalloc(&q, bytes);
    if (e == hipErrorOutOfMemory && !c->pool_idle.empty()) {
        pool_trim(c);
        e = hipMalloc(&q, bytes);
    }
    if (e != hipSuccess) return e;
    c->pool_live[q] = bytes;
    *p = static_cast<T *>(q);
    return hipSuccess;
}

template <typename T>
void tfree(mbpe_ctx *c, T *&p) {
    if (!p) return;
    auto it = c->pool_live.find((void *)p);
    if (it != c->pool_live.end()) {
        c->pool_idle.emplace(it->second, it->first);
        c->pool_live.erase(it);
    } else {
        (void)hipFree((void *)p);
    }
    p = nullptr;
}

template <typename T>
void trelease(mbpe_ctx *c, T *p) {
    if (!p) return;
    c->pool_live.erase((void *)p);
    (void)hipFree((void *)p);
}

void pool_trim(mbpe_ctx *c) {
    for (auto &kv : c->pool_idle) (void)hipFree(kv.second);
    c->pool_idle.clear();
}

int sync_ctl(mbpe_ctx *c) {
    HIPCHK(hipMemcpyAsync(&c->h_ctl, c->ctl, sizeof(DevCtl), hipMemcpyDeviceToHost, c->stream));
    HIPCHK(hipStreamSynchronize(c->stream));
    c->cur = (int)(c->h_ctl.cur & 1u);
#ifdef MBPE_DIAG
    if (getenv("MBPE_MERGE_DIAG") || getenv("MBPE_FUSED_DIAG")) c->h_ctl.err = 0;
#endif
    if (c->h_ctl.err) {
        char buf[320];
        snprintf(buf, sizeof(buf), "device error flags 0x%x (1=pair table full, 2=negative count, 4=missing pair, "
                                   "8=a pair occurs 2^31 times or more, or the byte-pair counts do not add up to the "
                                   "pairs scanned (a count reached 2^32), 16=a stream pass was skipped)",
                 c->h_ctl.err);
        mbpe_host::set_last_error(buf);
        return MBPE_ERR_OVERFLOW;
    }
    return MBPE_OK;
}

void free_training(mbpe_ctx *c) {
    tfree(c, c->tok[0]); tfree(c, c->tok[1]);
    tfree(c, c->sums); tfree(c, c->side); tfree(c, c->chg); tfree(c, c->tile_list);
    tfree(c, c->offsets);
    tfree(c, c->tab.hslot); tfree(c, c->tab.ekey); tfree(c, c->tab.ecnt); tfree(c, c->tab.cells);
    tfree(c, c->tab.bmax); tfree(c, c->tab.smax);
    tfree(c, c->ctl); tfree(c, c->best); tfree(c, c->xb); tfree(c, c->xb0); tfree(c, c->pair_cells);
    tfree(c, c->d_left); tfree(c, c->d_right); tfree(c, c->bs); tfree(c, c->sel); tfree(c, c->seq_flags); tfree(c, c->run_in);
    tfree(c, c->first_state);
    tfree(c, c->xf);
    tfree(c, c->wtok[0]); tfree(c, c->wtok[1]); tfree(c, c->wval); tfree(c, c->wscratch);
    tfree(c, c->wtab.keys); tfree(c, c->wtab.cnts); tfree(c, c->wctl); tfree(c, c->wbest); tfree(c, c->warg);
    tfree(c, c->wfs);
    c->wtab = {};
    c->wfirst = false;
    c->wide_active = false;
    c->wk = 0;
    c->wn_upper = 0;
    c->h_wbest.clear();
    c->LR = nullptr;
    c->pending = 0;
    c->begun = false;
    c->k = c->n_valid = 0;
    c->exhausted = false;
}

void free_corpus(mbpe_ctx *c) {
    dfree(c->d_text_owned);
    dfree(c->d_endmask);
    c->d_text = nullptr;
    c->loaded = false;
}

static inline bool dense_possible(const mbpe_ctx *c) { return c->vocab_size <= 32768; }
static inline bool use_dense(const mbpe_ctx *c) {
    if (!dense_possible(c)) return false;
    if (c->wide) return false;
    return c->opt_dense_table != 0;
}

int alloc_table_dense(mbpe_ctx *c) {
    uint32_t vshift = 8;
    while ((1u << vshift) < c->vocab_size) ++vshift;
    c->tab = {};
    c->tab.vshift = vshift;
    c->tab.ecap = 1u << (2 * vshift);
    const size_t cells = (size_t)1 << (2 * vshift);
    HIPCHK(tmalloc(c, &c->tab.cells, cells * 4));
    HIPCHK(hipMemsetAsync(c->tab.cells, 0, cells * 4, c->stream));
    const size_t nb = (cells >> kBlockShift) + 2, ns = (cells >> (2 * kBlockShift)) + 2;
    HIPCHK(tmalloc(c, &c->tab.bmax, nb * 8));
    HIPCHK(tmalloc(c, &c->tab.smax, ns * 8));
    HIPCHK(hipMemsetAsync(c->tab.bmax, 0, nb * 8, c->stream));
    HIPCHK(hipMemsetAsync(c->tab.smax, 0, ns * 8, c->stream));
    return MBPE_OK;
}

int alloc_table(mbpe_ctx *c, uint32_t ecap) {
    c->tab.ecap = ecap;
    c->hcap = next_pow2((uint64_t)ecap * 2);
    c->tab.hmask = c->hcap - 1;
    HIPCHK(tmalloc(c, &c->tab.hslot, (size_t)c->hcap * 8));
    HIPCHK(tmalloc(c, &c->tab.ekey, (size_t)ecap * 4));
    HIPCHK(tmalloc(c, &c->tab.ecnt, (size_t)ecap * 4));
    const size_t nb = ((size_t)ecap >> kBlockShift) + 2, ns = ((size_t)ecap >> (2 * kBlockShift)) + 2;
    HIPCHK(tmalloc(c, &c->tab.bmax, nb * 8));
    HIPCHK(tmalloc(c, &c->tab.smax, ns * 8));
    HIPCHK(hipMemsetAsync(c->tab.bmax, 0, nb * 8, c->stream));
    HIPCHK(hipMemsetAsync(c->tab.smax, 0, ns * 8, c->stream));
    launch_fill_u32(c->stream, reinterpret_cast<uint32_t *>(c->tab.hslot), (uint64_t)c->hcap * 2, 0xFFFFFFFFu);
    return MBPE_OK;
}

uint64_t batch_headroom(const mbpe_ctx *c, uint32_t steps) {
    uint64_t per = 2ull * c->vocab_size + 1;
    return per * steps;
}

uint64_t table_cap_limit(const mbpe_ctx *c) {
    uint64_t v = c->vocab_size;
    uint64_t lim = v * v;
    if (lim > (1ull << 30)) lim = 1ull << 30;
    return std::max<uint64_t>(lim, 1024);
}

struct WallTimer {
    float *acc;
    std::chrono::steady_clock::time_point t0 = std::chrono::steady_clock::now();
    explicit WallTimer(float *a) : acc(a) {}
    ~WallTimer() { *acc += std::chrono::duration<float, std::milli>(std::chrono::steady_clock::now() - t0).count(); }
};

int grow_table(mbpe_ctx *c, uint64_t want) {
    if (c->tab.cells) return MBPE_OK;
    WallTimer timer(&c->stats.ms_grow_table);
    c->stats.n_table_grows++;
    uint64_t lim = table_cap_limit(c);
    uint64_t ecap = std::min<uint64_t>(std::max<uint64_t>(want, (uint64_t)c->tab.ecap * 4), lim);
    if (ecap <= c->tab.ecap) return MBPE_OK;
    PairTable old = c->tab;
    c->tab = {};
    int rc = alloc_table(c, (uint32_t)ecap);
    if (rc != MBPE_OK) return rc;
    uint32_t n = c->h_ctl.n_entries;
    HIPCHK(hipMemcpyAsync(c->tab.ekey, old.ekey, (size_t)n * 4, hipMemcpyDeviceToDevice, c->stream));
    HIPCHK(hipMemcpyAsync(c->tab.ecnt, old.ecnt, (size_t)n * 4, hipMemcpyDeviceToDevice, c->stream));
    HIPCHK(hipMemcpyAsync(c->tab.bmax, old.bmax, (((size_t)old.ecap >> kBlockShift) + 2) * 8,
                          hipMemcpyDeviceToDevice, c->stream));
    HIPCHK(hipMemcpyAsync(c->tab.smax, old.smax, (((size_t)old.ecap >> (2 * kBlockShift)) + 2) * 8,
                          hipMemcpyDeviceToDevice, c->stream));
    launch_table_rehash(c->stream, c->tab, c->ctl);
    HIPCHK(hipStreamSynchronize(c->stream));
    trelease(c, old.hslot); trelease(c, old.ekey); trelease(c, old.ecnt);
    trelease(c, old.bmax); trelease(c, old.smax);
    return MBPE_OK;
}

int ensure_pc_scratch(mbpe_ctx *c) {
    if (!c->pc_scratch) HIPCHK(hipMalloc(&c->pc_scratch, pair_count_scratch_bytes(c->n_cus)));
    return MBPE_OK;
}

int ensure_events(std::vector<hipEvent_t> &pool, size_t n) {
    while (pool.size() < n) {
        hipEvent_t e;
        HIPCHK(hipEventCreate(&e));
        pool.push_back(e);
    }
    return MBPE_OK;
}

inline uint32_t endbit_of(const mbpe_ctx *c) { return !c->chunked ? 0u : c->barrier ? kBarrier : kEndBit; }

inline bool is_multi(const mbpe_ctx *c) { return c->n_ranks > 1 || c->opt_force_exchange; }

enum TokOrder { kBuffers01, kLiveFirst };

StreamView stream_view(const mbpe_ctx *c, TokOrder order) {
    const int first = order == kLiveFirst ? c->cur : 0;
    const bool multi = is_multi(c);
    StreamView v = {};
    v.stream = c->stream;
    v.tok = c->tok[first], v.tok_other = c->tok[1 - first];
    v.sums = c->sums, v.side = c->side, v.n_tiles = c->n_tiles;
    v.chg = c->chg, v.tile_list = c->tile_list;
    v.run_in = c->run_in, v.run_part = c->offsets + c->n_tiles;
    v.ctl = c->ctl;
    v.left_edge = multi ? c->d_left : nullptr, v.right_edge = multi ? c->d_right : nullptr;
    v.rank = c->rank, v.n_ranks = std::max(1, c->n_ranks);
    v.endbit = endbit_of(c), v.n_cus = c->n_cus;
    return v;
}

BatchView batch_view(const mbpe_ctx *c) { return BatchView{c->bs, c->hdr_m, c->hdr_adj, c->LR, c->pair_cells}; }

int do_compact(mbpe_ctx *c) {
    if (!c->n_tiles) return MBPE_OK;
    WallTimer timer(&c->stats.ms_compact);
    const int dst = 1 - c->cur;
    const StreamView v = stream_view(c, kLiveFirst);
    launch_tile_scan(v, c->offsets);
    launch_compact_scatter(v, c->offsets);
    const uint64_t live = c->h_ctl.n_live;
    const uint64_t padded = std::max<uint64_t>(round_up(live, kTile), kTile);
    launch_fill_u16(c->stream, c->tok[dst] + live, padded - live, (uint16_t)kHole);
    c->cur = dst;
    c->n_slots = padded;
    c->n_tiles = (uint32_t)(padded / kTile);
    launch_summarize(stream_view(c, kLiveFirst));
    DevCtl patch = c->h_ctl;
    patch.removed_total = 0;
    HIPCHK(hipMemcpyAsync(&c->ctl->removed_total, &patch.removed_total, sizeof(patch.removed_total),
                          hipMemcpyHostToDevice, c->stream));
    HIPCHK(hipMemsetD32Async(reinterpret_cast<hipDeviceptr_t>(&c->ctl->cur), c->cur, 1, c->stream));
    c->h_ctl.cur = (uint32_t)c->cur;
    HIPCHK(hipStreamSynchronize(c->stream));
    c->h_ctl.removed_total = 0;
    c->stats.n_compactions++;
    return MBPE_OK;
}

}

namespace mbpe_host {
int ctx_device(const mbpe_ctx *c) { return c->device; }
}

extern "C" {

int mbpe_create(int device_id, mbpe_ctx **out) {
    if (!out) { mbpe_host::set_last_error("mbpe_create: out is NULL"); return MBPE_ERR_ARG; }
    *out = nullptr;
    int n = 0;
    hipError_t e = hipGetDeviceCount(&n);
    if (e != hipSuccess || n <= 0 || device_id < 0 || device_id >= n) {
        mbpe_host::set_last_error("no usable HIP device (the MI355X path has no CPU fallback)");
        return MBPE_ERR_NO_DEVICE;
    }
    HIPCHK(hipSetDevice(device_id));
    mbpe_ctx *c = new mbpe_ctx();
    c->device = device_id;
    hipDeviceProp_t prop;
    if (hipGetDeviceProperties(&prop, device_id) == hipSuccess) c->n_cus = prop.multiProcessorCount;
    if (hipStreamCreateWithFlags(&c->stream, hipStreamNonBlocking) != hipSuccess ||
        hipEventCreate(&c->ev0) != hipSuccess || hipEventCreate(&c->ev1) != hipSuccess ||
        hipEventCreateWithFlags(&c->ev_sel, hipEventDisableTiming) != hipSuccess ||
        hipHostMalloc(reinterpret_cast<void **>(&c->h_seq), 64, hipHostMallocDefault) != hipSuccess) {
        mbpe_host::set_last_error("could not create HIP stream / events");
        delete c;
        return MBPE_ERR_HIP;
    }
    *out = c;
    return MBPE_OK;
}

void mbpe_destroy(mbpe_ctx *c) {
    if (!c) return;
    (void)hipSetDevice(c->device);
    if (c->stream) (void)hipStreamSynchronize(c->stream);
    free_training(c);
    pool_trim(c);
    free_corpus(c);
    dfree(c->pc_scratch);
    dfree(c->pc_bp);
    if (c->nccl_comm && rccl().ok) rccl().CommDestroy(c->nccl_comm);
    for (hipEvent_t e : c->kev) (void)hipEventDestroy(e);
    for (hipEvent_t e : c->kev_f) (void)hipEventDestroy(e);
    if (c->ev0) (void)hipEventDestroy(c->ev0);
    if (c->ev1) (void)hipEventDestroy(c->ev1);
    if (c->ev_sel) (void)hipEventDestroy(c->ev_sel);
    if (c->h_seq) (void)hipHostFree(c->h_seq);
    dfree(c->d_seq_info);
    if (c->stream) (void)hipStreamDestroy(c->stream);
    delete c;
}

int mbpe_set_option(mbpe_ctx *c, const char *name, int64_t value) {
    if (!c || !name) return MBPE_ERR_ARG;
    std::string n(name);
    if (n == "compact_den") c->opt_compact_den = value;
    else if (n == "batch") c->opt_batch = std::max<int64_t>(1, value);
    else if (n == "time_kernels") c->opt_time_kernels = value;
    else if (n == "force_exchange") c->opt_force_exchange = value;
    else if (n == "hier_argmax") c->opt_hier_argmax = value;
    else if (n == "multi_merge") c->opt_multi_merge = value;
    else if (n == "max_batch") c->opt_max_batch = std::min<int64_t>(std::max<int64_t>(1, value), kBatchMax);
    else if (n == "fused_min") c->opt_fused_min = std::max<int64_t>(2, value);
    else if (n == "dense_table") c->opt_dense_table = value;
    else if (n == "threshold_select") c->opt_threshold_select = value != 0;
    else if (n == "conflict_resolution") {
        if (value != 0 && value != 1) { mbpe_host::set_last_error("conflict_resolution: 0 = first, 1 = lexical"); return MBPE_ERR_ARG; }
        if (c->begun && (c->pending || (c->k < c->n_target && !c->exhausted))) {
            mbpe_host::set_last_error("conflict_resolution cannot change in the middle of a training");
            return MBPE_ERR_STATE;
        }
        c->opt_first = value == 0;
    }
    else if (n == "chunk_barrier") c->opt_barrier = value < 0 ? -1 : value != 0;
    else if (n == "first_batches") c->opt_first_batches = value != 0;
    else if (n == "sel_cap") c->opt_sel_cap = std::min<int64_t>(std::max<int64_t>(64, value), kSelCap);
    else if (n == "byte_table") c->opt_byte_table = value != 0;
    else if (n == "lockstep") c->opt_lockstep = value < 0 ? -1 : value != 0;
    else if (n == "pair_cells") c->opt_pair_cells = value < 0 ? -1 : value != 0;
    else if (n == "wide_from") c->opt_wide_from = value < 0 ? -1 : value;
    else if (n == "first_wide") c->opt_first_wide = value != 0;
    else if (n == "pc_repeat") c->opt_pc_repeat = std::min<int64_t>(std::max<int64_t>(1, value), 1000);
    else { mbpe_host::set_last_error("unknown option " + n); return MBPE_ERR_ARG; }
    return MBPE_OK;
}

int mbpe_load_corpus(mbpe_ctx *c, const uint8_t *text, uint64_t n_bytes, const uint64_t *chunk_off,
                     uint64_t n_chunks, int text_on_device) {
    if (!c || (!text && n_bytes)) { mbpe_host::set_last_error("mbpe_load_corpus: NULL argument"); return MBPE_ERR_ARG; }
    HIPCHK(hipSetDevice(c->device));
    free_training(c);
    free_corpus(c);
    if (n_bytes != c->n_bytes || (chunk_off != nullptr) != c->chunked) pool_trim(c);
    c->n_bytes = n_bytes;
    c->chunked = chunk_off != nullptr;
    c->n_chunks = chunk_off ? n_chunks : 1;
    c->n_barriers = 0;
    c->barrier = false;
    c->inert = false;
    if (chunk_off) {
        if (chunk_off[0] != 0 || chunk_off[n_chunks] != n_bytes) {
            mbpe_host::set_last_error("chunk_off must start at 0 and end at n_bytes");
            return MBPE_ERR_ARG;
        }
        for (uint64_t i = 0; i < n_chunks; ++i)
            if (chunk_off[i] > chunk_off[i + 1]) {
                mbpe_host::set_last_error("chunk_off must be ascending");
                return MBPE_ERR_ARG;
            }
    }
    if (text_on_device && ((uintptr_t)text & 15)) {
        mbpe_host::set_last_error("device text must be 16-byte aligned");
        return MBPE_ERR_ARG;
    }

    std::vector<uint8_t> tmp;
    const uint8_t *h_text = text;
    if (text_on_device && n_bytes) {
        bool need_all = chunk_off != nullptr;
        uint64_t take = need_all ? n_bytes : std::min<uint64_t>(n_bytes, 64);
        tmp.resize(take);
        HIPCHK(hipMemcpy(tmp.data(), text, take, hipMemcpyDeviceToHost));
        h_text = tmp.data();
    }
    const uint64_t n_vec = (n_bytes + 15) / 16;
    std::vector<uint8_t> mask;
    if (chunk_off) {
        mask.assign(n_vec * 2 + 16, 0);
        uint64_t dropped = 0;
        for (uint64_t ci = 0; ci < n_chunks; ++ci) {
            uint64_t s = chunk_off[ci], e = chunk_off[ci + 1];
            if (e == s) continue;
            mask[(e - 1) >> 3] |= (uint8_t)(1u << ((e - 1) & 7));
            if (h_text[s] == 0 && stoi_parses(h_text + s + 1, e - s - 1)) {
                for (uint64_t i = s; i < e; ++i) mask[i >> 3] |= (uint8_t)(1u << (i & 7));
                dropped++;
            }
        }
        c->n_chunks = n_chunks - dropped;
        uint64_t ends = 0;
        for (uint8_t b : mask) ends += (uint64_t)__builtin_popcount(b);
        c->n_barriers = ends;
    } else if (n_bytes && h_text[0] == 0) {
        uint64_t have = text_on_device ? tmp.size() : n_bytes;
        bool parses = stoi_parses(h_text + 1, have - 1);
        if (!parses && text_on_device && have < n_bytes) {
            bool all_ws = true;
            for (uint64_t i = 1; i < have; ++i)
                if (!(h_text[i] == ' ' || (h_text[i] >= 9 && h_text[i] <= 13))) { all_ws = false; break; }
            if (all_ws) {
                tmp.resize(n_bytes);
                HIPCHK(hipMemcpy(tmp.data(), text, n_bytes, hipMemcpyDeviceToHost));
                parses = stoi_parses(tmp.data() + 1, n_bytes - 1);
            }
        }
        c->inert = parses;
        if (parses) c->n_chunks = 0;
    }

    if (text_on_device) {
        c->d_text = text;
    } else {
// ... 53 lines not shown
        w += ends[i] - starts[i];
    }
    off[n_chunks] = w;
    return mbpe_load_corpus(c, buf.data(), packed, off.data(), n_chunks, 0);
}

static uint64_t pairs_scanned(const mbpe_ctx *c) {
    if (c->chunked) return c->n_bytes - c->n_barriers;
    return c->inert || c->n_bytes < 2 ? 0 : c->n_bytes - 1;
}

int mbpe_pair_count_u8(mbpe_ctx *c, uint32_t *table65536_out) {
    if (!c) return MBPE_ERR_ARG;
    if (!c->loaded) { mbpe_host::set_last_error("mbpe_pair_count_u8: no corpus loaded"); return MBPE_ERR_STATE; }
    HIPCHK(hipSetDevice(c->device));
    int rcs = ensure_pc_scratch(c);
    if (rcs != MBPE_OK) return rcs;
    if (!c->pc_bp) HIPCHK(hipMalloc(&c->pc_bp, 65536 * 4 + 16));
    uint32_t *bp = c->pc_bp;
    HIPCHK(hipMemsetAsync(bp, 0, 65536 * 4, c->stream));
    const int reps = table65536_out ? 1 : (int)std::max<int64_t>(1, c->opt_pc_repeat);
    rcs = ensure_events(c->kev, 2ull * reps);
    if (rcs != MBPE_OK) return rcs;
    HIPCHK(hipEventRecord(c->ev0, c->stream));
    if (!c->inert)
        for (int r = 0; r < reps; ++r)
            launch_pair_count_u8(c->stream, c->d_text, c->n_bytes, c->d_endmask, bp, c->n_cus, c->pc_scratch,
                                 c->kev[2 * r], c->kev[2 * r + 1]);
    HIPCHK(hipEventRecord(c->ev1, c->stream));
    unsigned long long *sum_dev = reinterpret_cast<unsigned long long *>(bp + 65536);
    if (reps == 1) launch_pair_total(c->stream, bp, nullptr, 0, sum_dev, nullptr);
    hipError_t e = hipStreamSynchronize(c->stream);
    if (e == hipSuccess) e = hipGetLastError();
    if (e == hipSuccess && table65536_out) e = hipMemcpy(table65536_out, bp, 65536 * 4, hipMemcpyDeviceToHost);
    unsigned long long sum = 0;
    if (e == hipSuccess && reps == 1) e = hipMemcpy(&sum, sum_dev, 8, hipMemcpyDeviceToHost);
    if (e != hipSuccess) { mbpe_host::set_last_error(hip_err("pair count", e)); return MBPE_ERR_HIP; }
    if (reps == 1 && sum != pairs_scanned(c)) {
        mbpe_host::set_last_error("mbpe_pair_count_u8: the counts add up to " + std::to_string(sum) + " of " +
                                  std::to_string(pairs_scanned(c)) + " pairs: a pair occurs 2^32 times or more");
        return MBPE_ERR_OVERFLOW;
    }
    HIPCHK(hipEventElapsedTime(&c->stats.ms_pair_count, c->ev0, c->ev1));
    c->stats.ms_pair_count /= (float)reps;
    c->stats.ms_pair_count_kernel = 0;
    if (!c->inert && c->n_bytes >= 2) {
        float sum = 0;
        for (int r = 0; r < reps; ++r) {
            float km = 0;
            HIPCHK(hipEventElapsedTime(&km, c->kev[2 * r], c->kev[2 * r + 1]));
            sum += km;
        }
        c->stats.ms_pair_count_kernel = sum / (float)reps;
    }
    c->stats.pair_count_launches += (uint32_t)reps;
#ifdef MBPE_PC_STAMPS
    {
        std::vector<unsigned long long> st((size_t)c->n_cus * 16);
        HIPCHK(hipMemcpy(st.data(), reinterpret_cast<const char *>(c->pc_scratch) + (size_t)c->n_cus * 32768 * 4, st.size() * 8,
                         hipMemcpyDeviceToHost));
        unsigned long long t0 = ~0ull;
        for (int w = 0; w < c->n_cus; ++w) if (st[16 * w] && st[16 * w] < t0) t0 = st[16 * w];
        for (int k = 0; k < 16; ++k) {
            double lo = 1e30, hi = 0, sum = 0; int cnt = 0;
            for (int w = 0; w < c->n_cus; ++w) {
                if (!st[16 * w + k]) continue;
                const double us = (double)(st[16 * w + k] - t0) * 0.01;
                lo = std::min(lo, us); hi = std::max(hi, us); sum += us; ++cnt;
            }
            if (cnt) fprintf(stderr, "pc stamp %2d: min %8.2f avg %8.2f max %8.2f us (%d workgroups)\n", k, lo, sum / cnt, hi, cnt);
        }
    }
#endif
    return MBPE_OK;
}


static inline bool use_hier(const mbpe_ctx *c) {
    if (c->opt_hier_argmax >= 0) return c->opt_hier_argmax != 0;
    if (c->tab.cells) return c->tab.ecap > (1u << 20);
    return c->h_ctl.n_entries > (1u << 20);
}

static int begin_local(mbpe_ctx *c, uint32_t vocab_size) {
    free_training(c);
    c->vocab_size = vocab_size;
    c->n_target = vocab_size - 256;
    c->k = 0;
    c->n_valid = 0;
    c->exhausted = false;
    c->first_legacy = false;
    c->sel_attempts = 3;
    c->merges_per_seq = 0;
    c->first_b = c->first_s = 0;

    const uint64_t n = c->inert ? 0 : c->n_bytes;
    const uint64_t n_bar = c->barrier ? c->n_barriers : 0;
    const uint64_t dense_slots = std::max<uint64_t>(round_up(n + n_bar, kTile), kTile);
    c->n_slots = c->barrier ? std::max<uint64_t>(2 * round_up(n, kTile / 2), kTile) : dense_slots;
    c->cap_slots = dense_slots;
    if (c->n_slots / kTile > 0x0FFFFFF0ull) { mbpe_host::set_last_error("corpus shard too large"); return MBPE_ERR_ARG; }
    c->n_tiles = (uint32_t)(c->n_slots / kTile);
    c->hdr_words = exchange_header_words(c->n_ranks);
    c->max_batch_eff = (uint32_t)std::min<int64_t>(c->opt_max_batch, is_multi(c) ? 1024 : kBatchMax);
    c->adj_pitch = (uint32_t)round_up(std::max<uint32_t>(c->max_batch_eff, 64u), 64);
    c->hdrb_words = (batch_header_words(c->adj_pitch) + 3) / 4 * 4;
    HIPCHK(tmalloc(c, &c->tok[0], c->n_slots * 2));
    HIPCHK(tmalloc(c, &c->tok[1], c->cap_slots * 2));
    HIPCHK(tmalloc(c, &c->sums, (size_t)c->n_tiles * sizeof(TileSum)));
    HIPCHK(tmalloc(c, &c->side, (size_t)c->n_tiles * sizeof(TileSum)));
    HIPCHK(tmalloc(c, &c->chg, ((size_t)c->n_tiles / 32 + 2) * 4));
    HIPCHK(tmalloc(c, &c->tile_list, ((size_t)c->n_tiles + 64) * 4));
    HIPCHK(hipMemsetAsync(c->chg, 0, ((size_t)c->n_tiles / 32 + 2) * 4, c->stream));
    HIPCHK(tmalloc(c, &c->offsets, ((size_t)c->n_tiles + tile_scan_scratch(c->n_tiles)) * 8));
    const size_t xb_words = (size_t)c->hdr_words + c->hdrb_words + lr_words(vocab_size, c->max_batch_eff) + 8;
    const size_t xb0_words = 65536 + (size_t)c->hdr_words + kPairCountWords;
    HIPCHK(tmalloc(c, &c->xb, xb_words * 4));
    HIPCHK(tmalloc(c, &c->xb0, xb0_words * 4));
    HIPCHK(hipMemsetAsync(c->xb, 0, xb_words * 4, c->stream));
    HIPCHK(hipMemsetAsync(c->xb0, 0, xb0_words * 4, c->stream));
    if (c->opt_pair_cells > 0 || (c->opt_pair_cells < 0 && c->n_slots >= (64ull << 20))) {
        const size_t cells = (size_t)c->max_batch_eff * 65536u;
        HIPCHK(tmalloc(c, &c->pair_cells, cells * 4));
        HIPCHK(hipMemsetAsync(c->pair_cells, 0, cells * 4, c->stream));
    }
    c->hdr_m = c->xb + c->hdr_words;
    c->hdr_adj = c->hdr_m + kBatchMax;
    c->LR = c->xb + c->hdr_words + c->hdrb_words;
    HIPCHK(tmalloc(c, &c->bs, sizeof(BatchState)));
    HIPCHK(tmalloc(c, &c->sel, sizeof(SelList)));
    HIPCHK(tmalloc(c, &c->run_in, ((size_t)c->n_tiles + 64) * 4));
    HIPCHK(tmalloc(c, &c->seq_flags, 4096 * 4 * 4));
    HIPCHK(hipMemsetAsync(c->bs, 0, sizeof(BatchState), c->stream));
    if (c->opt_first) {
        HIPCHK(tmalloc(c, &c->first_state, first_state_bytes()));
        launch_first_init(c->stream, c->first_state);
        if (is_multi(c)) {
            HIPCHK(tmalloc(c, &c->xf, (size_t)c->hdr_words * 4));
            HIPCHK(hipMemsetAsync(c->xf, 0, (size_t)c->hdr_words * 4, c->stream));
        }
    }
    c->k_upper = 0;
    HIPCHK(tmalloc(c, &c->d_left, sizeof(RankEdge)));
    HIPCHK(tmalloc(c, &c->d_right, sizeof(RankEdge)));
    HIPCHK(tmalloc(c, &c->ctl, sizeof(DevCtl)));
    HIPCHK(tmalloc(c, &c->best, ((size_t)c->n_target + 2) * 8));
    {
        DevCtl init = {};
        init.n_live = n + n_bar;
        init.n_ranks = (uint32_t)std::max(1, c->n_ranks);
        init.first_mode = c->opt_first ? 1u : 0u;
        init.adj_pitch = c->adj_pitch;
        init.cells_on = c->pair_cells ? 1u : 0u;
        init.cells_min = c->opt_pair_cells > 0 ? 2u : kCellsMinBatch;
        c->h_ctl = init;
        HIPCHK(hipMemcpyAsync(c->ctl, &c->h_ctl, sizeof(DevCtl), hipMemcpyHostToDevice, c->stream));
    }
    HIPCHK(hipMemsetAsync(c->best, 0, ((size_t)c->n_target + 2) * 8, c->stream));

    uint64_t want = 65536 + 2 * batch_headroom(c, (uint32_t)c->opt_batch);
    want = std::max<uint64_t>(want, n / 8);
    want = std::min<uint64_t>(want, table_cap_limit(c));
    int rc = use_dense(c) ? alloc_table_dense(c) : alloc_table(c, (uint32_t)want);
    if (rc != MBPE_OK) return rc;

    rc = ensure_pc_scratch(c);
    if (rc != MBPE_OK) return rc;
    pool_trim(c);
    HIPCHK(hipEventRecord(c->ev0, c->stream));
    if (n >= 2) launch_pair_count_u8(c->stream, c->d_text, n, c->d_endmask, c->xb0, c->n_cus, c->pc_scratch);
    c->cur = 0;
    if (c->barrier) {
        launch_widen_barrier(c->stream, c->d_text, n, c->d_endmask, c->tok[0], c->n_slots);
        launch_summarize(stream_view(c, kLiveFirst));
        const double ms_compact = c->stats.ms_compact;
        rc = do_compact(c);
        if (rc != MBPE_OK) return rc;
        c->stats.n_compactions--;
        c->stats.ms_compact = ms_compact;
        tfree(c, c->tok[0]);
        pool_trim(c);
        HIPCHK(tmalloc(c, &c->tok[0], c->cap_slots * 2));
    } else {
        launch_widen(c->stream, c->d_text, n, c->d_endmask, c->tok[0], c->n_slots);
        launch_summarize(stream_view(c, kLiveFirst));
    }
    if (is_multi(c)) {
        uint32_t *hdr = c->xb0 + 65536;
        launch_rank_edge(stream_view(c, kLiveFirst), hdr);
        const uint64_t p = pairs_scanned(c);
        for (uint32_t i = 0; i < kPairCountWords; ++i) c->h_pcount[i] = (uint32_t)(p >> (16 * i)) & 0xFFFFu;
        HIPCHK(hipMemcpyAsync(hdr + c->hdr_words, c->h_pcount, sizeof(c->h_pcount), hipMemcpyHostToDevice, c->stream));
    }
    return MBPE_OK;
}

static void update_hot_possible(mbpe_ctx *c, unsigned long long top_count, uint64_t merges) {
    c->last_top = top_count;
    if (c->comm_external) { c->hot_possible = 1; return; }
    const unsigned long long live = c->h_ctl.n_live;
    const unsigned long long eaten = merges * top_count;
    c->hot_possible = !(live > eaten && top_count * 8192ull < (live - eaten) * (unsigned long long)std::max(1, c->n_ranks));
}

static inline bool first_sharded(const mbpe_ctx *c) { return c->opt_first && is_multi(c); }

static void first_tiebreak(mbpe_ctx *c, unsigned long long *best, int seq, int phase) {
    launch_first_tiebreak(stream_view(c, seq ? kBuffers01 : kLiveFirst), c->tab, best, c->first_state, c->xf, seq, phase);
}

static void begin_finish_a(mbpe_ctx *c) {
    const uint32_t endbit = endbit_of(c);
    if (is_multi(c)) {
        uint32_t *hdr = c->xb0 + 65536;
        launch_boundary_pairs(c->stream, c->xb0, hdr, c->n_ranks, endbit, hdr + c->hdr_words);
        launch_compose_edges(c->stream, hdr, c->rank, c->n_ranks, c->d_left, c->d_right);
        launch_pair_total(c->stream, c->xb0, hdr + c->hdr_words, 0, nullptr, c->ctl);
    } else {
        launch_pair_total(c->stream, c->xb0, nullptr, pairs_scanned(c), nullptr, c->ctl);
    }
    launch_table_init(c->stream, c->xb0, c->tab, c->ctl);
    launch_argmax(c->stream, c->tab, c->ctl, c->best, use_hier(c));
    if (c->opt_first) first_tiebreak(c, c->best, 0, first_sharded(c) ? 1 : 0);
}

static int begin_finish_b(mbpe_ctx *c) {
    if (first_sharded(c)) first_tiebreak(c, c->best, 0, 2);
    HIPCHK(hipEventRecord(c->ev1, c->stream));
    int rc = sync_ctl(c);
    if (rc != MBPE_OK) return rc;
    HIPCHK(hipGetLastError());
    HIPCHK(hipEventElapsedTime(&c->stats.ms_begin, c->ev0, c->ev1));
    unsigned long long b0 = 0;
    HIPCHK(hipMemcpy(&b0, c->best, 8, hipMemcpyDeviceToHost));
    c->exhausted = (b0 == 0);
    update_hot_possible(c, b0 >> 32, (uint64_t)std::max<int64_t>(c->opt_batch, 1) * kBatchMax);
    c->begun = true;
// ... 499 lines not shown
                }
                rc = after_batch(c);
                if (rc != MBPE_OK) return rc;
                break;
            }
        }
        done += batch;
        rc = after_batch(c);
        if (rc != MBPE_OK) return rc;
    }
    if (steps_done_out) *steps_done_out = done;
    return MBPE_OK;
}


static int wide_alloc_table(mbpe_ctx *c, WideTable *t, uint64_t want_entries) {
    uint32_t bits = 12;
    while ((1ull << bits) < 2 * want_entries && bits < 31) ++bits;
    if ((1ull << bits) < 2 * want_entries) { mbpe_host::set_last_error("pair table beyond 2^30 entries"); return MBPE_ERR_OVERFLOW; }
    *t = {};
    t->mask = (uint32_t)((1ull << bits) - 1);
    t->shift = 64 - bits;
    HIPCHK(tmalloc(c, &t->keys, (size_t)8 << bits));
    HIPCHK(tmalloc(c, &t->cnts, (size_t)4 << bits));
    launch_wide_table_clear(c->stream, *t);
    return MBPE_OK;
}

static uint64_t wide_headroom(unsigned long long top, uint32_t merges) { return (uint64_t)merges * (2ull * top + 2); }

static int wide_sync(mbpe_ctx *c) {
    HIPCHK(hipMemcpyAsync(&c->h_wctl, c->wctl, sizeof(WideCtl), hipMemcpyDeviceToHost, c->stream));
    HIPCHK(hipStreamSynchronize(c->stream));
    HIPCHK(hipGetLastError());
    if (c->h_wctl.err) {
        mbpe_host::set_last_error("device error: the 32-bit pair table is full");
        return MBPE_ERR_OVERFLOW;
    }
    return MBPE_OK;
}

static int wide_convert(mbpe_ctx *c) {
    int rc = sync_ctl(c);
    if (rc != MBPE_OK) return rc;
    rc = do_compact(c);
    if (rc != MBPE_OK) return rc;
    const uint64_t n_live_slots = c->h_ctl.n_live;
    const uint64_t n_tok = n_live_slots - (c->barrier ? c->n_barriers : 0);
    const uint32_t n_wide = c->n_target_total - c->n_target;
    HIPCHK(tmalloc(c, &c->wtok[0], std::max<uint64_t>(n_tok, 1) * 4));
    HIPCHK(tmalloc(c, &c->wtok[1], std::max<uint64_t>(n_tok, 1) * 4));
    HIPCHK(tmalloc(c, &c->wval, std::max<uint64_t>(n_live_slots, 1) * 4));
    HIPCHK(tmalloc(c, &c->wscratch, wide_scratch_words(n_live_slots) * 4));
    HIPCHK(tmalloc(c, &c->wctl, sizeof(WideCtl)));
    HIPCHK(tmalloc(c, &c->wbest, ((size_t)n_wide + 2) * sizeof(WideBest)));
    HIPCHK(tmalloc(c, &c->warg, 2 * 1024 * 8));
    HIPCHK(hipMemsetAsync(c->wctl, 0, sizeof(WideCtl), c->stream));
    c->wfirst = c->opt_first != 0;
    if (c->wfirst) {
        HIPCHK(tmalloc(c, &c->wfs, sizeof(WideFirst)));
        HIPCHK(hipMemsetAsync(c->wfs, 0, sizeof(WideFirst), c->stream));
        HIPCHK(hipMemsetAsync(&c->wfs->pos, 0xFF, sizeof(c->wfs->pos), c->stream));
        HIPCHK(hipMemsetD32Async(reinterpret_cast<hipDeviceptr_t>(&c->wctl->first), 1, 1, c->stream));
    }
    const uint32_t barrier = c->barrier ? kBarrier : 0xFFFFFFFFu;
    const uint32_t endbit = c->chunked && !c->barrier ? kEndBit : 0u;
    launch_wide_from_slots(c->stream, c->tok[c->cur], n_live_slots, barrier, endbit, c->wval, c->wscratch, c->wtok[0], c->wctl);
    c->wcur = 0;
    unsigned long long top = c->last_top == ~0ull ? n_tok : c->last_top;
    rc = wide_alloc_table(c, &c->wtab, (uint64_t)c->h_ctl.n_entries + wide_headroom(top, 16));
    if (rc != MBPE_OK) return rc;
    launch_wide_table_from16(c->stream, c->tab.ekey, c->tab.ecnt, c->h_ctl.n_entries, c->wtab, c->wctl);
    rc = wide_sync(c);
    if (rc != MBPE_OK) return rc;
    if (c->h_wctl.n != n_tok || c->h_wctl.n_entries != c->h_ctl.n_entries) {
        mbpe_host::set_last_error("conversion to 32-bit tokens lost tokens or pairs");
        return MBPE_ERR_OVERFLOW;
    }
    c->wn_upper = n_tok;
    c->wk = 0;
    c->h_wbest.clear();
    c->wide_active = true;
    tfree(c, c->tok[0]); tfree(c, c->tok[1]); tfree(c, c->sums); tfree(c, c->side); tfree(c, c->chg); tfree(c, c->tile_list);
    tfree(c, c->offsets); tfree(c, c->run_in); tfree(c, c->xb); tfree(c, c->pair_cells);
    tfree(c, c->tab.hslot); tfree(c, c->tab.ekey); tfree(c, c->tab.ecnt); tfree(c, c->tab.bmax); tfree(c, c->tab.smax);
    tfree(c, c->first_state);
    c->LR = nullptr;
    pool_trim(c);
    return MBPE_OK;
}

static int wide_steps(mbpe_ctx *c, uint32_t n_steps, uint32_t *done_out) {
    *done_out = 0;
    const uint32_t n_wide = c->n_target_total - c->n_target;
    uint32_t done = 0;
    unsigned long long top = c->h_wbest.empty() ? (c->last_top == ~0ull ? c->wn_upper : c->last_top)
                                                : (unsigned long long)c->h_wbest.back().count;
    while (done < n_steps && c->wk < n_wide) {
        const uint32_t group = std::min<uint32_t>({16u, n_steps - done, n_wide - c->wk});
        if (2 * ((uint64_t)c->h_wctl.n_entries + wide_headroom(top, group)) > (uint64_t)c->wtab.mask + 1) {
            WideTable old = c->wtab;
            int rc = wide_alloc_table(c, &c->wtab, 2 * ((uint64_t)c->h_wctl.n_entries + wide_headroom(top, group)));
            if (rc != MBPE_OK) return rc;
            HIPCHK(hipMemsetD32Async(reinterpret_cast<hipDeviceptr_t>(&c->wctl->n_entries), 0, 1, c->stream));
            launch_wide_rehash(c->stream, old, c->wtab, c->wctl);
            HIPCHK(hipStreamSynchronize(c->stream));
            trelease(c, old.keys); trelease(c, old.cnts);
            c->stats.n_table_grows++;
        }
        HIPCHK(hipMemsetD32Async(reinterpret_cast<hipDeviceptr_t>(&c->wctl->k_limit), (int)(c->wk + group), 1, c->stream));
        HIPCHK(hipEventRecord(c->ev0, c->stream));
        for (uint32_t g = 0; g < group; ++g) {
            launch_wide_argmax(c->stream, c->wtab, c->wctl, c->wbest, c->warg);
            if (c->wfirst)
                launch_wide_first(c->stream, c->wtok[c->wcur ^ (g & 1)], c->wn_upper, c->wtab, c->wctl, c->wbest, c->warg,
                                  c->wfs);
            launch_wide_merge(c->stream, c->wtok[c->wcur ^ (g & 1)], c->wtok[c->wcur ^ (g & 1) ^ 1], c->wn_upper, c->wval,
                              c->wscratch, c->wtab, c->wctl, 256 + c->n_target);
        }
        HIPCHK(hipEventRecord(c->ev1, c->stream));
        int rc = wide_sync(c);
        if (rc != MBPE_OK) return rc;
        float ms = 0;
        HIPCHK(hipEventElapsedTime(&ms, c->ev0, c->ev1));
        c->stats.ms_steps += ms;
        const uint32_t ran = c->h_wctl.k - c->wk;
        if (ran == 0) break;
        c->h_wbest.resize((size_t)c->wk + ran);
        HIPCHK(hipMemcpy(c->h_wbest.data() + c->wk, c->wbest + c->wk, (size_t)ran * sizeof(WideBest), hipMemcpyDeviceToHost));
        c->wcur ^= (int)(ran & 1u);
        c->wn_upper = c->h_wctl.n;
        c->wk += ran;
        done += ran;
        top = (unsigned long long)std::max(0, c->h_wbest.back().count);
        if (!c->wfirst && c->h_wbest.back().count == 0 && done < n_steps && c->wk < n_wide) {
            const uint32_t fill = std::min<uint32_t>(n_steps - done, n_wide - c->wk);
            c->h_wbest.resize((size_t)c->wk + fill, c->h_wbest.back());
            c->wk += fill;
            done += fill;
            HIPCHK(hipMemsetD32Async(reinterpret_cast<hipDeviceptr_t>(&c->wctl->k), (int)c->wk, 1, c->stream));
            HIPCHK(hipStreamSynchronize(c->stream));
            c->h_wctl.k = c->wk;
        }
        if (ran < group) break;
    }
    *done_out = done;
    return MBPE_OK;
}

int mbpe_train_sequences(mbpe_ctx *c, uint32_t n_sequences, uint32_t *merges_done_out) {
    if (merges_done_out) *merges_done_out = 0;
    if (!c) return MBPE_ERR_ARG;
    if (!c->begun) { mbpe_host::set_last_error("mbpe_train_sequences before mbpe_train_begin"); return MBPE_ERR_STATE; }
    if (c->pending || (is_multi(c) && c->comm_external)) {
        mbpe_host::set_last_error("mbpe_train_sequences: not available with an external transport (use mbpe_train_steps)");
        return MBPE_ERR_STATE;
    }
    if (c->wide_active || (c->wide && c->k >= c->n_target))
        return mbpe_train_steps(c, n_sequences, merges_done_out);
    if (!use_batches(c)) return mbpe_train_steps(c, n_sequences, merges_done_out);
    HIPCHK(hipSetDevice(c->device));
    return train_steps_batched(c, c->n_target, merges_done_out, n_sequences);
}

int mbpe_comm_exchange_buffer(mbpe_ctx *c, void **dev_ptr_out, uint64_t *n_u32_out) {
    if (!c || !dev_ptr_out || !n_u32_out) return MBPE_ERR_ARG;
// ... 69 lines not shown
        c->pending = 4;
        return MBPE_NEED_EXCHANGE;
    }
    if (c->pending == 4) {
        c->pending = 0;
        seq_stage_c(c);
        int rc = sync_ctl(c);
        if (rc != MBPE_OK) return rc;
        HIPCHK(hipGetLastError());
        const uint32_t before = c->k;
        c->k = c->h_ctl.k_done;
        rc = after_batch(c);
        if (rc != MBPE_OK) return rc;
        if (c->k < c->pending_target && c->k != before) {
            if (!c->tab.cells && (uint64_t)c->h_ctl.n_entries + seq_headroom(c) > c->tab.ecap) {
                rc = grow_table(c, ((uint64_t)c->h_ctl.n_entries + seq_headroom(c)) * 2);
                if (rc != MBPE_OK) return rc;
            }
            c->k_upper = c->k;
            rc = seq_stage_a(c, -1);
            if (rc != MBPE_OK) return rc;
            HIPCHK(hipStreamSynchronize(c->stream));
            c->pending = 3;
            return MBPE_NEED_EXCHANGE;
        }
        return MBPE_OK;
    }
    mbpe_host::set_last_error("no exchange pending");
    return MBPE_ERR_STATE;
}

int mbpe_train_result(mbpe_ctx *c, uint32_t *merges_out, int32_t *counts_out, uint32_t cap_merges,
                      uint32_t *n_merges_out) {
    if (!c) return MBPE_ERR_ARG;
    if (!c->begun) { mbpe_host::set_last_error("mbpe_train_result before mbpe_train_begin"); return MBPE_ERR_STATE; }
    HIPCHK(hipSetDevice(c->device));
    uint32_t n = c->exhausted ? 0 : c->n_valid;
    std::vector<unsigned long long> h(n);
    if (n) HIPCHK(hipMemcpy(h.data(), c->best, (size_t)n * 8, hipMemcpyDeviceToHost));
    if (c->opt_first) {
        uint32_t real = 0;
        while (real < n && (h[real] >> 32) != 0) ++real;
        n = real;
    }
    const uint32_t nw = c->wide_active ? (uint32_t)c->h_wbest.size() : 0u;
    if (n_merges_out) *n_merges_out = n + nw;
    if (n + nw > cap_merges && merges_out) { mbpe_host::set_last_error("merges_out too small"); return MBPE_ERR_ARG; }
    if (!(n + nw) || !merges_out) return MBPE_OK;
    for (uint32_t i = 0; i < n; ++i) {
        uint32_t key = ~(uint32_t)h[i];
        merges_out[2 * i] = key >> 16;
        merges_out[2 * i + 1] = key & 0xFFFFu;
        if (counts_out) counts_out[i] = (int32_t)(h[i] >> 32);
    }
    for (uint32_t i = 0; i < nw; ++i) {
        merges_out[2 * (n + i)] = c->h_wbest[i].first;
        merges_out[2 * (n + i) + 1] = c->h_wbest[i].second;
        if (counts_out) counts_out[n + i] = c->h_wbest[i].count;
    }
    return MBPE_OK;
}

int mbpe_get_stats(mbpe_ctx *c, mbpe_stats *out) {
    if (!c || !out) return MBPE_ERR_ARG;
    c->stats.n_slots = c->begun ? c->n_slots : 0;
    c->stats.n_live = c->begun ? c->h_ctl.n_live - (c->barrier ? c->n_barriers : 0) : 0;
    c->stats.n_merges = c->exhausted ? 0 : c->n_valid;
    c->stats.n_pairs = c->begun ? c->h_ctl.n_entries : 0;
    c->stats.n_batches = c->begun ? (use_batches(c) ? c->h_ctl.n_batches : c->k) : 0;
    c->stats.n_fused = c->begun ? c->h_ctl.n_fused : 0;
    c->stats.n_fused_dropped = c->begun ? c->h_ctl.n_fused_dropped : 0;
    c->stats.cut_conflict = c->begun ? c->h_ctl.cut_conflict : 0;
    c->stats.cut_bucket = c->begun ? c->h_ctl.cut_bucket : 0;
    c->stats.cut_single = c->begun ? c->h_ctl.cut_single : 0;
    c->stats.cut_full = c->begun ? c->h_ctl.cut_full : 0;
    c->stats.n_validation_drops = c->begun ? c->h_ctl.n_validation_drops : 0;
    c->stats.n_sel_fallback = c->begun ? c->h_ctl.n_sel_fallback : 0;
    c->stats.n_sel_retry = c->begun ? c->h_ctl.n_sel_retry : 0;
    c->stats.adapt_limit = c->begun ? c->h_ctl.adapt_limit : 0;
    c->stats.n_sel_blocks = c->begun ? c->h_ctl.n_sel_blocks : 0;
    for (int i = 0; i < 8; ++i) c->stats.size_hist[i] = c->begun ? c->h_ctl.size_hist[i] : 0;
    c->stats.n_skipped = c->begun ? c->h_ctl.n_skipped : 0;
    c->stats.n_skip_cut = c->begun ? c->h_ctl.n_skip_cut : 0;
    if (c->begun && c->wide_active) {
        c->stats.n_slots = c->h_wctl.n;
        c->stats.n_live = c->h_wctl.n;
        c->stats.n_merges += (uint32_t)c->h_wbest.size();
        c->stats.n_pairs = c->h_wctl.n_entries;
        c->stats.n_batches += c->wk;
    }
    *out = c->stats;
    return MBPE_OK;
}

int mbpe_train(mbpe_ctx *c, const uint8_t *text, uint64_t n_bytes, const uint64_t *chunk_off, uint64_t n_chunks,
               uint32_t vocab_size, int conflict_resolution, uint32_t *merges_out, int32_t *counts_out,
               uint32_t *n_merges_out, mbpe_stats *stats_out) {
    if (!c || !merges_out) { mbpe_host::set_last_error("mbpe_train: NULL argument"); return MBPE_ERR_ARG; }
    if (conflict_resolution != 0 && conflict_resolution != 1) {
        mbpe_host::set_last_error("conflict_resolution: 0 = first, 1 = lexical");
        return MBPE_ERR_ARG;
    }
    int rc = mbpe_load_corpus(c, text, n_bytes, chunk_off, n_chunks, 0);
    if (rc != MBPE_OK) return rc;
    const int64_t keep = c->opt_first;
    c->opt_first = conflict_resolution == 0;
    rc = mbpe_train_begin(c, vocab_size);
    if (rc == MBPE_OK) rc = mbpe_train_steps(c, vocab_size - 256, nullptr);
    if (rc == MBPE_OK) rc = mbpe_train_result(c, merges_out, counts_out, vocab_size - 256, n_merges_out);
    if (rc == MBPE_OK && stats_out) mbpe_get_stats(c, stats_out);
    c->opt_first = keep;
    return rc;
}

int mbpe_train_lexical(mbpe_ctx *c, const uint8_t *text, uint64_t n_bytes, const uint64_t *chunk_off,
                       uint64_t n_chunks, uint32_t vocab_size, uint32_t *merges_out, int32_t *counts_out,
                       uint32_t *n_merges_out, mbpe_stats *stats_out) {
    return mbpe_train(c, text, n_bytes, chunk_off, n_chunks, vocab_size, 1, merges_out, counts_out, n_merges_out,
                      stats_out);
}

int mbpe_get_stream(mbpe_ctx *c, uint32_t *tokens_out, uint8_t *chunk_end_out, uint64_t cap, uint64_t *n_out) {
    if (!c || !n_out) return MBPE_ERR_ARG;
    if (!c->begun) { mbpe_host::set_last_error("mbpe_get_stream before mbpe_train_begin"); return MBPE_ERR_STATE; }
    HIPCHK(hipSetDevice(c->device));
    HIPCHK(hipStreamSynchronize(c->stream));
    if (c->wide_active) {
        const uint64_t n = c->h_wctl.n;
        *n_out = n;
        if (!tokens_out) return MBPE_OK;
        if (cap < n) { mbpe_host::set_last_error("tokens_out too small"); return MBPE_ERR_ARG; }
        if (n) HIPCHK(hipMemcpy(tokens_out, c->wtok[c->wcur], n * 4, hipMemcpyDeviceToHost));
        for (uint64_t i = 0; i < n; ++i) {
            if (chunk_end_out) chunk_end_out[i] = c->chunked ? (uint8_t)(tokens_out[i] >> 31) : 0;
            tokens_out[i] &= kTokIdMask;
        }
        return MBPE_OK;
    }
    std::vector<uint16_t> h(c->n_slots);
    HIPCHK(hipMemcpy(h.data(), c->tok[c->cur], c->n_slots * 2, hipMemcpyDeviceToHost));
    const bool endflag = c->chunked && !c->barrier;
    const uint32_t idmask = endflag ? 0x7FFFu : 0xFFFFu;
    uint64_t w = 0;
    for (uint64_t i = 0; i < c->n_slots; ++i) {
        if (h[i] == kHole) continue;
        if (c->barrier && h[i] == kBarrier) {
            if (tokens_out && chunk_end_out && w) chunk_end_out[w - 1] = 1;
            continue;
        }
        if (tokens_out) {
            if (w >= cap) { mbpe_host::set_last_error("tokens_out too small"); return MBPE_ERR_ARG; }
            tokens_out[w] = h[i] & idmask;
            if (chunk_end_out) chunk_end_out[w] = endflag ? (h[i] >> 15) & 1 : 0;
        }
        ++w;
    }
    *n_out = w;
    return MBPE_OK;
}

int mbpe_stream_device(mbpe_ctx *c, const void **slots_out, uint64_t *n_slots_out, uint32_t *slot_bits_out,
                       uint32_t *end_bit_out, uint32_t *barrier_out) {
    if (!c || !slots_out || !n_slots_out) return MBPE_ERR_ARG;
    if (!c->begun) { mbpe_host::set_last_error("mbpe_stream_device before mbpe_train_begin"); return MBPE_ERR_STATE; }
    HIPCHK(hipSetDevice(c->device));
    if (c->wide_active) {
// ... 177 lines not shown
```

### minbpe-cc_amd/python/mbpe/__init__.py

```python
import ctypes
import os

import numpy as np

_PKG_DIR = os.path.dirname(os.path.dirname(os.path.dirname(os.path.abspath(__file__))))
LIB_PATH = os.environ.get("MBPE_LIB") or os.path.join(_PKG_DIR, "libmbpe.so")

OK = 0
NEED_EXCHANGE = 1
ERR_ARG, ERR_NO_DEVICE, ERR_HIP, ERR_VOCAB, ERR_STATE = -1, -2, -3, -4, -5
ERR_OOM, ERR_REGEX, ERR_SPLIT_GAP, ERR_COMM, ERR_OVERFLOW, ERR_IO = -6, -7, -8, -9, -10, -11
COMM_ID_BYTES = 128

EXPORTS = [
    "mbpe_last_error", "mbpe_version", "mbpe_create", "mbpe_destroy", "mbpe_load_corpus",
    "mbpe_pair_count_u8", "mbpe_train_begin", "mbpe_train_steps", "mbpe_train_sequences", "mbpe_train_result",
    "mbpe_train_lexical", "mbpe_train", "mbpe_get_stats", "mbpe_get_stream", "mbpe_stream_device", "mbpe_table_device", "mbpe_get_pairs", "mbpe_compact",
    "mbpe_set_option", "mbpe_comm_unique_id", "mbpe_comm_init", "mbpe_comm_init_external",
    "mbpe_comm_exchange_buffer", "mbpe_comm_exchange_done", "mbpe_presplit",
    "mbpe_split_count", "mbpe_split_offsets", "mbpe_split_has_gaps", "mbpe_split_starts", "mbpe_split_ends",
    "mbpe_split_free", "mbpe_load_corpus_ranges", "mbpe_split_pattern", "mbpe_encode_chunks",
    "mbpe_encode_chunks_device", "mbpe_decoder_create", "mbpe_decoder_destroy", "mbpe_decode_tokens",
    "mbpe_decode_slots", "mbpe_decoder_kernel_ms", "mbpe_decode_stream", "mbpe_encoder_create",
    "mbpe_encoder_destroy", "mbpe_encoder_encode", "mbpe_encoder_set_option", "mbpe_encoder_kernel_ms",
    "mbpe_encoder_alloc_count", "mbpe_encoder_pass_tokens", "mbpe_decode_batch", "mbpe_decoder_alloc_count",
    "mbpe_pack_tokens", "mbpe_unpack_tokens", "mbpe_pack_kernel_ms", "mbpe_encoder_encode_batch", "mbpe_encoder_pack_ms",
]
TOK_EXPORTS = [
    "mbpe_tok_create", "mbpe_tok_destroy", "mbpe_tok_set_special_tokens", "mbpe_tok_train", "mbpe_tok_set_merges",
    "mbpe_tok_get_merges", "mbpe_tok_save", "mbpe_tok_load", "mbpe_tok_encode", "mbpe_tok_encode_device",
    "mbpe_tok_decode", "mbpe_tok_decode_device", "mbpe_tok_encode_batch_device", "mbpe_tok_decode_batch_device",
    "mbpe_tok_encode_batch_packed_device", "mbpe_tok_decode_padded_device",
]


class Stats(ctypes.Structure):
    _fields_ = [
        ("n_bytes", ctypes.c_uint64), ("n_chunks", ctypes.c_uint64), ("n_slots", ctypes.c_uint64),
        ("n_live", ctypes.c_uint64), ("n_merges", ctypes.c_uint32), ("n_compactions", ctypes.c_uint32),
        ("n_pairs", ctypes.c_uint64), ("ms_pair_count", ctypes.c_float), ("ms_begin", ctypes.c_float),
        ("ms_steps", ctypes.c_float), ("pair_count_launches", ctypes.c_uint32), ("merge_launches", ctypes.c_uint32),
        ("ms_merge_kernel", ctypes.c_float), ("n_batches", ctypes.c_uint32),
        ("n_fused", ctypes.c_uint32), ("n_fused_dropped", ctypes.c_uint32), ("cut_conflict", ctypes.c_uint32),
        ("cut_bucket", ctypes.c_uint32), ("cut_single", ctypes.c_uint32), ("cut_full", ctypes.c_uint32),
        ("n_validation_drops", ctypes.c_uint32), ("ms_grow_table", ctypes.c_float), ("ms_compact", ctypes.c_float),
        ("n_table_grows", ctypes.c_uint32), ("n_sel_fallback", ctypes.c_uint32),
        ("fused_launches", ctypes.c_uint32), ("ms_fused_kernel", ctypes.c_float), ("fused_slots", ctypes.c_uint64),
        ("n_sel_retry", ctypes.c_uint32), ("adapt_limit", ctypes.c_uint32), ("n_sel_blocks", ctypes.c_uint64), ("size_hist", ctypes.c_uint32 * 8),
        ("n_skipped", ctypes.c_uint32), ("n_skip_cut", ctypes.c_uint32),
        ("exchange_words", ctypes.c_uint64), ("exchanges", ctypes.c_uint32), ("pad_", ctypes.c_uint32),
        ("fused_live_tokens", ctypes.c_uint64), ("ms_pair_count_kernel", ctypes.c_float), ("pad2_", ctypes.c_uint32),
    ]

    def as_dict(self):
        d = {k: getattr(self, k) for k, _ in self._fields_}
        d["size_hist"] = list(self.size_hist)
        return d



PACK_PADDED, PACK_PACKED = 0, 1
NO_TOKEN = 0xFFFFFFFF


class PackSpec(ctypes.Structure):
    _fields_ = [
        ("layout", ctypes.c_uint32), ("seq_len", ctypes.c_uint32), ("out_bits", ctypes.c_uint32),
        ("pad_id", ctypes.c_uint32), ("bos_id", ctypes.c_uint32), ("eos_id", ctypes.c_uint32),
        ("pad_left", ctypes.c_uint32), ("trunc_left", ctypes.c_uint32),
    ]


_ID_DTYPES = {16: np.uint16, 32: np.uint32, 64: np.uint64}


def pack_spec(seq_len, layout="padded", out_bits=32, pad_id=0, bos_id=None, eos_id=None, pad_left=False,
              trunc_left=False):
    if isinstance(layout, str):
        if layout not in ("padded", "packed"):
            raise ValueError("layout must be \"padded\" or \"packed\"")
        layout = PACK_PADDED if layout == "padded" else PACK_PACKED
    return PackSpec(layout, seq_len, out_bits, pad_id, NO_TOKEN if bos_id is None else bos_id,
                    NO_TOKEN if eos_id is None else eos_id, int(bool(pad_left)), int(bool(trunc_left)))


class MbpeError(RuntimeError):
    def __init__(self, code, msg):
        super().__init__("mbpe error %d: %s" % (code, msg))
        self.code = code


_lib = None


def lib():
    global _lib
    if _lib is not None:
        return _lib
    if not os.path.exists(LIB_PATH):
        raise ImportError("libmbpe.so is not built (%s); run __graft_entry__.build()" % LIB_PATH)
    L = ctypes.CDLL(LIB_PATH)
    vp, u64, u32, i32, i64 = ctypes.c_void_p, ctypes.c_uint64, ctypes.c_uint32, ctypes.c_int, ctypes.c_int64
    L.mbpe_last_error.restype = ctypes.c_char_p
    L.mbpe_version.restype = ctypes.c_char_p
    L.mbpe_create.argtypes = [i32, ctypes.POINTER(vp)]
    L.mbpe_destroy.argtypes = [vp]
    L.mbpe_destroy.restype = None
    L.mbpe_load_corpus.argtypes = [vp, vp, u64, vp, u64, i32]
    L.mbpe_pair_count_u8.argtypes = [vp, vp]
    L.mbpe_train_begin.argtypes = [vp, u32]
    L.mbpe_train_steps.argtypes = [vp, u32, vp]
    L.mbpe_train_sequences.argtypes = [vp, u32, vp]
    L.mbpe_train_result.argtypes = [vp, vp, vp, u32, vp]
    L.mbpe_train_lexical.argtypes = [vp, vp, u64, vp, u64, u32, vp, vp, vp, vp]
    L.mbpe_train.argtypes = [vp, vp, u64, vp, u64, u32, i32, vp, vp, vp, vp]
    L.mbpe_get_stats.argtypes = [vp, vp]
    L.mbpe_get_stream.argtypes = [vp, vp, vp, u64, vp]
    L.mbpe_stream_device.argtypes = [vp, ctypes.POINTER(vp), ctypes.POINTER(u64), ctypes.POINTER(u32), ctypes.POINTER(u32),
                                     ctypes.POINTER(u32)]
    L.mbpe_table_device.argtypes = [vp, ctypes.POINTER(vp), ctypes.POINTER(u32)]
    L.mbpe_get_pairs.argtypes = [vp, vp, vp, vp, u64, vp]
    L.mbpe_compact.argtypes = [vp]
    L.mbpe_set_option.argtypes = [vp, ctypes.c_char_p, i64]
    L.mbpe_comm_unique_id.argtypes = [vp]
    L.mbpe_comm_init.argtypes = [vp, vp, i32, i32]
    L.mbpe_comm_init_external.argtypes = [vp, i32, i32]
    L.mbpe_comm_exchange_buffer.argtypes = [vp, ctypes.POINTER(vp), ctypes.POINTER(u64)]
    L.mbpe_comm_exchange_done.argtypes = [vp]
    L.mbpe_presplit.argtypes = [ctypes.c_char_p, vp, u64, ctypes.POINTER(vp)]
    L.mbpe_split_count.argtypes = [vp]
    L.mbpe_split_count.restype = u64
    L.mbpe_split_offsets.argtypes = [vp]
    L.mbpe_split_offsets.restype = ctypes.POINTER(ctypes.c_uint64)
    L.mbpe_split_has_gaps.argtypes = [vp]
# ... 734 lines not shown
```

Measured before the change: 80340 merges/s.

## Defer slow-halo and rename-needing tiles to a separate fused slow kernel

Adds a DEFER variant of the fused batch kernel. Tiles that would need the slow halo path or a token rename are appended to a slow list through an atomic counter instead of being handled inline, and a separate k_fused_slow kernel then processes only the listed tiles with the full TT and rename logic. The goal is to keep the common path free of divergent slow-halo and TT-rename branches, and to skip the TT build in the main kernel when the byte LUT is active. In exchange each batch launches extra kernels and pays atomic list traffic, and the feature switches itself off when more than 1/8 of tiles are deferred.

```diff
diff --git a/include/mbpe.h b/include/mbpe.h
--- a/include/mbpe.h
+++ b/include/mbpe.h
@@ -73,7 +73,8 @@
     uint32_t pad_;
     uint64_t fused_live_tokens;
     float    ms_pair_count_kernel;
-    uint32_t pad2_;
+    uint32_t slow_tiles_off;
+    uint64_t n_slow_tiles;
 } mbpe_stats;
 
 MBPE_API const char *mbpe_last_error(void);
diff --git a/minbpe-cc_amd/csrc/kernels.hip b/minbpe-cc_amd/csrc/kernels.hip
--- a/minbpe-cc_amd/csrc/kernels.hip
+++ b/minbpe-cc_amd/csrc/kernels.hip
@@ -1666,6 +1666,7 @@
     BatchLutMem *m;
     uint32_t mul;
     bool bytes;
+    bool marks = false;
     uint32_t idmask;
     __device__ __forceinline__ BatchLut(BatchLutMem *mem, const BatchState *bs, uint32_t idmask_)
         : m(mem), mul(rfl(bs->hash_mul)), bytes(rfl(bs->byte_lut) != 0u), idmask(idmask_) {}
@@ -2391,7 +2392,7 @@
     return __ballot(need) != 0ull || hneed;
 }
 
-template <int MODE, int DIAG, bool WRITE, bool TT, class DC>
+template <int MODE, int DIAG, bool WRITE, bool TT, bool MARKS, class DC>
 __device__ __forceinline__ uint4 fused_tile_pf(const uint4 q_orig, const uint32_t s[8], const Halo h,
                                                uint32_t old_x, uint32_t old_y, uint32_t old_z, const BatchLut &lut,
                                                uint32_t X0, uint32_t tile, TileSum *sout, uint32_t *hdr_adj, uint32_t *LR,
@@ -2461,7 +2462,7 @@
             uint32_t rm_unused = 0;
             bool ws_unused = false, no_rename = false;
             if (TT) tt_rename<MODE>(s, h, ti, run_in[tile]);
-            fused_tile_pf<MODE, 0, false, TT>(t0.q, s, h, rlane(t0.smw, 4), rlane(t0.smw, 5), rlane(t0.smw, 6), lut,
+            fused_tile_pf<MODE, 0, false, TT, false>(t0.q, s, h, rlane(t0.smw, 4), rlane(t0.smw, 5), rlane(t0.smw, 6), lut,
                                               256u + ctl_k_done, tile, nullptr, hdr_adj, LR, dc, dc_on, rm_unused, ws_unused,
                                               lr_rsrc, adj_pitch, nullptr, chg, TT, &ti, no_rename, t_rsrc, use_t);
         }
@@ -2477,7 +2478,7 @@
     }
 }
 
-template <int MODE, int DIAG, bool WRITE, bool TT, class DC>
+template <int MODE, int DIAG, bool WRITE, bool TT, bool MARKS, class DC>
 __device__ __forceinline__ uint4 fused_tile_pf(const uint4 q_orig, const uint32_t s[8], const Halo h,
                                                uint32_t old_x, uint32_t old_y, uint32_t old_z, const BatchLut &lut,
                                                uint32_t X0, uint32_t tile, TileSum *sout, uint32_t *hdr_adj, uint32_t *LR,
@@ -2511,8 +2512,8 @@
 #pragma unroll
     for (int j = 0; j < 7; ++j) n[j] = s[j + 1];
     n[7] = wave_from_next(s[0], h.n1);
-    const uint32_t ef = lane == 0 ? h.p1 : lane == 1 ? h.p2 : lane == 2 ? tile_last : (TT && lane == 3) ? h.n1 : kHole;
-    const uint32_t es = (lane == 0 ? tile_first : lane == 1 ? h.p1 : (TT && lane == 3) ? h.n2 : h.n1) & idmask;
+    const uint32_t ef = lane == 0 ? h.p1 : lane == 1 ? h.p2 : lane == 2 ? tile_last : ((TT || MARKS) && lane == 3) ? h.n1 : kHole;
+    const uint32_t es = (lane == 0 ? tile_first : lane == 1 ? h.p1 : ((TT || MARKS) && lane == 3) ? h.n2 : h.n1) & idmask;
     uint32_t idx[8], eidx;
     if (lut.bytes) {
 #pragma unroll
@@ -2532,11 +2533,20 @@
             }
             eidx = lane == 3 ? kNone : eidx;
         }
+        if (MARKS) {
+            if (lut.marks) {
+                bool mark = eidx == kTTMark;
+#pragma unroll
+                for (int j = 0; j < 8; ++j) mark = mark || idx[j] == kTTMark;
+                if (__ballot(mark) != 0ull) { need_rename = true; return q_orig; }
+            }
+            eidx = lane == 3 ? kNone : eidx;
+        }
     } else {
         uint32_t Hm = 0, Wm = 0;
         {
             bool second_key;
-            const bool hit = pair_hit2(lut, ef, es, second_key) && !(TT && lane == 3);
+            const bool hit = pair_hit2(lut, ef, es, second_key) && !((TT || MARKS) && lane == 3);
             Hm = hit ? 1u : 0u;
             Wm = second_key ? 1u : 0u;
         }
@@ -2676,7 +2686,12 @@
 #ifndef MBPE_FUSED_WAVES
 #define MBPE_FUSED_WAVES 4
 #endif
-template <int MODE, bool HOT, bool TT, int DIAG = 0>
+#ifndef MBPE_SLOW_MAX_DIV
+#define MBPE_SLOW_MAX_DIV 8
+#endif
+__device__ __forceinline__ bool defer_with_tt(const BatchState *bs) { return bs->tt_index != kNoTT && bs->byte_lut == 0u; }
+
+template <int MODE, bool HOT, bool TT, int DIAG = 0, bool DEFER = false>
 __global__ __launch_bounds__(kLutThreads, MBPE_FUSED_WAVES * 256 / kLutThreads) void k_fused_batch(uint16_t *tok0, uint16_t *tok1,
                                                                const TileSum *__restrict__ sin,
                                                                TileSum *__restrict__ sout, uint32_t n_tiles,
@@ -2684,7 +2699,8 @@
                                                                uint32_t *hdr_adj, uint32_t *LR, DevCtl *ctl,
                                                                const RankEdge *le, const RankEdge *re,
                                                                uint32_t *hdr_m, const uint32_t *__restrict__ run_in,
-                                                               int hot_launched, uint32_t *T) {
+                                                               int hot_launched, uint32_t *T,
+                                                               uint32_t *__restrict__ slow_list) {
     constexpr uint32_t idmask = MODE == 1 ? 0x7FFFu : 0xFFFFu;
     __shared__ BatchLutMem lut_mem;
     const uint32_t lane = lane_id();
@@ -2693,7 +2709,8 @@
     __shared__ DeltaCacheSmall dc;
     const uint32_t n_keys = ctl->batch_n;
     if (n_keys < 2 || !ctl->fused) return;
-    if ((bs->tt_index != kNoTT) != TT) return;
+    if ((ctl->slow_on != 0u) != DEFER) return;
+    if ((DEFER ? defer_with_tt(bs) : bs->tt_index != kNoTT) != TT) return;
     __shared__ TTInfo ti;
     __shared__ __attribute__((aligned(16))) uint16_t stage_mem[kLutThreads / kWave][kTileSlots];
     uint16_t *stage = stage_mem[threadIdx.x / kWave];
@@ -2704,7 +2721,8 @@
     constexpr bool dc_on = HOT;
     if (dc_on) dc_init(dc);
     BatchLut lut(&lut_mem, bs, idmask);
-    lut_build(lut, bs, n_keys, idmask - 1u, TT);
+    lut_build(lut, bs, n_keys, idmask - 1u, TT || DEFER);
+    if (DEFER && !TT) lut.marks = lut.bytes && rfl(bs->tt_index) != kNoTT;
     if (TT) tt_build(ti, bs, n_keys, idmask - 1u);
     if (blockIdx.x == 0 && threadIdx.x == 0) ctl->marks_all = 1;
     uint32_t tile = rfl(blockIdx.x * waves_per_block + threadIdx.x / kWave);
@@ -2733,10 +2751,127 @@
 
         uint4 outq = t0.q;
         bool wrote_sum = false;
+        bool defer = false;
         const uint32_t old_x = rlane(t0.smw, 4), old_y = rlane(t0.smw, 5), old_z = rlane(t0.smw, 6);
         if (DIAG == 4) {
             asm volatile("" :: "v"(t0.smw));
         } else if ((old_z & 0xFFFFu) != 0) {
+            uint32_t s[8];
+            unpack8(t0.q, s);
+            Halo h;
+            const uint32_t pw1 = rlane(t0.smw, 1), pw2 = rlane(t0.smw, 2);
+            const uint32_t nw0 = rlane(t0.smw, 8), nw2 = rlane(t0.smw, 10);
+            const bool fast = tile > 0 && tile + 1 < n_tiles && (pw2 & 0xFFFFu) >= 2 && (nw2 & 0xFFFFu) >= 2;
+            if (DEFER) {
+                h.p1 = pw1 >> 16; h.p2 = pw1 & 0xFFFFu;
+                h.n1 = nw0 & 0xFFFFu; h.n2 = nw0 >> 16;
+                defer = !fast;
+            } else if (fast) {
+                h.p1 = pw1 >> 16; h.p2 = pw1 & 0xFFFFu;
+                h.n1 = nw0 & 0xFFFFu; h.n2 = nw0 >> 16;
+            } else {
+                h = halo_slow(sin, n_tiles, tile, le, re);
+            }
+            bool renamed = false;
+            bool need_rename = false;
+            if (TT && !lut.bytes && !(DEFER && defer)) {
+                uint32_t nx[8];
+#pragma unroll
+                for (int j = 0; j < 7; ++j) nx[j] = s[j + 1];
+                nx[7] = wave_from_next(s[0], h.n1);
+                const uint32_t li = (old_z & 0xFFFFu) - 1u;
+                const bool mine = lane == (li >> 3);
+#pragma unroll
+                for (uint32_t j = 0; j < 8; ++j)
+                    if ((li & 7u) == j) nx[j] = mine ? h.n1 : nx[j];
+                const int lrem = (int)(old_z & 0xFFFFu) - (int)(lane * 8u);
+                const uint32_t lm = lrem >= 8 ? 0xFFu : lrem <= 0 ? 0u : (1u << lrem) - 1u;
+                if (tt_needed<MODE>(s, nx, h, old_x & 0xFFFFu, ti, lm)) {
+                    tt_rename<MODE>(s, h, ti, run_in[tile]);
+                    renamed = true;
+                }
+            }
+            if (!DEFER || !defer)
+                outq = fused_tile_pf<MODE, DIAG, true, TT, DEFER && !TT>(t0.q, s, h, old_x, old_y, old_z, lut, X0, tile, sout, hdr_adj,
+                                                                  LR, dc, dc_on, wave_rm, wrote_sum, lr_rsrc, adj_pitch, stage,
+                                                                  chg, renamed, &ti, need_rename, t_rsrc, use_t);
+            if (DEFER && !TT) defer = defer || need_rename;
+            if (TT && need_rename && !(DEFER && defer)) {
+                tt_rename<MODE>(s, h, ti, run_in[tile]);
+                outq = fused_tile_pf<MODE, DIAG, true, TT, false>(t0.q, s, h, old_x, old_y, old_z, lut, X0, tile, sout, hdr_adj, LR,
+                                                           dc, dc_on, wave_rm, wrote_sum, lr_rsrc, adj_pitch, stage, chg, true,
+                                                           &ti, need_rename, t_rsrc, use_t);
+            }
+        }
+        if (DEFER && defer) {
+            if (lane == 0) {
+                const uint32_t at = atomicAdd(&ctl->slow_n, 1u);
+                if (at < n_tiles) slow_list[at] = tile;
+            }
+        } else {
+        if (!wrote_sum && lane == 0) reinterpret_cast<uint4 *>(sout)[tile] = make_uint4(old_x, old_y, old_z, 0u);
+        MBPE_GLOBAL_AS char *obase =
+            (MBPE_GLOBAL_AS char *)uniform_ptr(reinterpret_cast<uintptr_t>(dst) + (uint64_t)tile * (kWave * 16u));
+        u32x4 oq; oq.x = outq.x; oq.y = outq.y; oq.z = outq.z; oq.w = outq.w;
+        __builtin_nontemporal_store(oq, (MBPE_GLOBAL_AS u32x4 *)(obase + lane * 16u));
+        }
+
+        if (!v1) break;
+        tile += n_waves;
+#pragma unroll
+        for (int d = 0; d + 1 < kDepth; ++d) ring[d] = ring[d + 1];
+        ring[kDepth - 1] = t_new;
+    }
+    }
+    if (dc_on) dc_flush(dc, LR);
+    if (lane == 0 && wave_rm) atomicAdd(&ctl->rm, wave_rm);
+    if (TT) {
+        tt_flush(ti, hdr_m);
+    }
+}
+
+template <int MODE>
+__global__ __launch_bounds__(kLutThreads) void k_fused_slow(uint16_t *tok0, uint16_t *tok1, const TileSum *__restrict__ sin,
+                                                            TileSum *__restrict__ sout, uint32_t n_tiles,
+                                                            uint32_t *__restrict__ chg, const BatchState *bs,
+                                                            uint32_t *hdr_adj, uint32_t *LR, DevCtl *ctl,
+                                                            const RankEdge *le, const RankEdge *re, uint32_t *hdr_m,
+                                                            const uint32_t *__restrict__ run_in, uint32_t *T,
+                                                            const uint32_t *__restrict__ slow_list) {
+    constexpr uint32_t idmask = MODE == 1 ? 0x7FFFu : 0xFFFFu;
+    __shared__ BatchLutMem lut_mem;
+    __shared__ TTInfo ti;
+    __shared__ __attribute__((aligned(16))) uint16_t stage_mem[kLutThreads / kWave][kTileSlots];
+    const uint32_t waves_per_block = kLutThreads / kWave;
+    const uint32_t n_list = ctl->slow_n < n_tiles ? ctl->slow_n : n_tiles;
+    if (blockIdx.x * waves_per_block >= n_list) return;
+    const uint32_t n_keys = ctl->batch_n;
+    const uint32_t lane = lane_id();
+    const uint32_t n_waves = gridDim.x * waves_per_block;
+    uint16_t *stage = stage_mem[threadIdx.x / kWave];
+    const uint16_t *tok = ctl->cur ? tok1 : tok0;
+    uint16_t *dst = ctl->cur ? tok0 : tok1;
+    const uint32_t X0 = 256u + ctl->k_done;
+    BatchLut lut(&lut_mem, bs, idmask);
+    lut_build(lut, bs, n_keys, idmask - 1u, true);
+    tt_build(ti, bs, n_keys, idmask - 1u);
+    const __amdgpu_buffer_rsrc_t sums_rsrc =
+        __builtin_amdgcn_make_buffer_rsrc(const_cast<TileSum *>(sin), 0, n_tiles * 16u, 0x00020000);
+    const __amdgpu_buffer_rsrc_t lr_rsrc = __builtin_amdgcn_make_buffer_rsrc(LR, 0, 0xFFFFFFFCu, 0x00020000);
+    const bool use_t = T != nullptr && !dc_wanted(bs->packed[0] >> 32, ctl->n_live * ctl->n_ranks) && ctl->cells_on != 0u &&
+                       n_keys >= ctl->cells_min;
+    const __amdgpu_buffer_rsrc_t t_rsrc = __builtin_amdgcn_make_buffer_rsrc(T ? T : LR, 0, T ? 0xFFFFFFFCu : 0u, 0x00020000);
+    const uint32_t adj_pitch = rfl(ctl->adj_pitch);
+    DeltaCacheSmall no_dc;
+    uint32_t wave_rm = 0;
+    for (uint32_t i = rfl(blockIdx.x * waves_per_block + threadIdx.x / kWave); i < n_list; i += n_waves) {
+        const uint32_t tile = rfl(slow_list[i]);
+        if (tile >= n_tiles) continue;
+        const TileIn t0 = tile_issue(tok, sums_rsrc, tile);
+        uint4 outq = t0.q;
+        bool wrote_sum = false;
+        const uint32_t old_x = rlane(t0.smw, 4), old_y = rlane(t0.smw, 5), old_z = rlane(t0.smw, 6);
+        if ((old_z & 0xFFFFu) != 0) {
             uint32_t s[8];
             unpack8(t0.q, s);
             Halo h;
@@ -2751,7 +2886,7 @@
             }
             bool renamed = false;
             bool need_rename = false;
-            if (TT && !lut.bytes) {
+            if (!lut.bytes) {
                 uint32_t nx[8];
 #pragma unroll
                 for (int j = 0; j < 7; ++j) nx[j] = s[j + 1];
@@ -2768,34 +2903,21 @@
                     renamed = true;
                 }
             }
-            outq = fused_tile_pf<MODE, DIAG, true, TT>(t0.q, s, h, old_x, old_y, old_z, lut, X0, tile, sout, hdr_adj, LR, dc,
-                                                       dc_on, wave_rm, wrote_sum, lr_rsrc, adj_pitch, stage, chg, renamed, &ti,
-                                                       need_rename, t_rsrc, use_t);
-            if (TT && need_rename) {
+            outq = fused_tile_pf<MODE, 0, true, true, false>(t0.q, s, h, old_x, old_y, old_z, lut, X0, tile, sout, hdr_adj, LR,
+                                                             no_dc, false, wave_rm, wrote_sum, lr_rsrc, adj_pitch, stage, chg,
+                                                             renamed, &ti, need_rename, t_rsrc, use_t);
+            if (need_rename) {
                 tt_rename<MODE>(s, h, ti, run_in[tile]);
-                outq = fused_tile_pf<MODE, DIAG, true, TT>(t0.q, s, h, old_x, old_y, old_z, lut, X0, tile, sout, hdr_adj, LR,
-                                                           dc, dc_on, wave_rm, wrote_sum, lr_rsrc, adj_pitch, stage, chg, true,
-                                                           &ti, need_rename, t_rsrc, use_t);
+                outq = fused_tile_pf<MODE, 0, true, true, false>(t0.q, s, h, old_x, old_y, old_z, lut, X0, tile, sout, hdr_adj,
+                                                                 LR, no_dc, false, wave_rm, wrote_sum, lr_rsrc, adj_pitch, stage,
+                                                                 chg, true, &ti, need_rename, t_rsrc, use_t);
             }
         }
         if (!wrote_sum && lane == 0) reinterpret_cast<uint4 *>(sout)[tile] = make_uint4(old_x, old_y, old_z, 0u);
-        MBPE_GLOBAL_AS char *obase =
-            (MBPE_GLOBAL_AS char *)uniform_ptr(reinterpret_cast<uintptr_t>(dst) + (uint64_t)tile * (kWave * 16u));
-        u32x4 oq; oq.x = outq.x; oq.y = outq.y; oq.z = outq.z; oq.w = outq.w;
-        __builtin_nontemporal_store(oq, (MBPE_GLOBAL_AS u32x4 *)(obase + lane * 16u));
-
-        if (!v1) break;
-        tile += n_waves;
-#pragma unroll
-        for (int d = 0; d + 1 < kDepth; ++d) ring[d] = ring[d + 1];
-        ring[kDepth - 1] = t_new;
-    }
-    }
-    if (dc_on) dc_flush(dc, LR);
+        reinterpret_cast<uint4 *>(dst)[(uint64_t)tile * kWave + lane] = outq;
+    }
     if (lane == 0 && wave_rm) atomicAdd(&ctl->rm, wave_rm);
-    if (TT) {
-        tt_flush(ti, hdr_m);
-    }
+    tt_flush(ti, hdr_m);
 }
 
 __global__ __launch_bounds__(256) void k_pair_cells_fold(uint32_t *__restrict__ T, uint32_t *__restrict__ LR, const DevCtl *ctl) {
@@ -3292,7 +3414,7 @@
         bool no_rename = false;
         DeltaCacheSmall no_dc;
         if (TT) tt_rename<MODE>(s, h, ti, run_in[tile]);
-        const uint4 qn = fused_tile_pf<MODE, 2, true, TT>(t0.q, s, h, rlane(t0.smw, 4), rlane(t0.smw, 5), rlane(t0.smw, 6), lut,
+        const uint4 qn = fused_tile_pf<MODE, 2, true, TT, false>(t0.q, s, h, rlane(t0.smw, 4), rlane(t0.smw, 5), rlane(t0.smw, 6), lut,
                                                           X0, tile, sout, nullptr, nullptr, no_dc, false, rm, wrote,
                                                           __amdgpu_buffer_rsrc_t(), 0u, stage, chg, TT, &ti, no_rename);
         if (wrote) {
@@ -3311,7 +3433,7 @@
     if (lane == 0 && wave_rm) atomicAdd(&ctl->rm, wave_rm);
 }
 
-__global__ void k_seq_finish(DevCtl *ctl, uint32_t *fused_flag, const BatchState *bs) {
+__global__ void k_seq_finish(DevCtl *ctl, uint32_t *fused_flag, const BatchState *bs, uint32_t n_tiles) {
     if (blockIdx.x || threadIdx.x) return;
     const uint32_t bs_skip_n = bs->skip_n;
     const uint32_t rm_seq = ctl->batch_n >= 2 ? ctl->rm : 0u;
@@ -3342,6 +3464,12 @@
         ctl->cell_hits * 2ull < (unsigned long long)rm_seq)
         ctl->cells_on = 0;
     ctl->cell_hits = 0;
+    ctl->n_slow_tiles += ctl->slow_n;
+    if (ctl->slow_on == 1u && (unsigned long long)ctl->slow_n * (unsigned long long)MBPE_SLOW_MAX_DIV > n_tiles) {
+        ctl->slow_on = 0;
+        ctl->slow_off = 1;
+    }
+    ctl->slow_n = 0;
     if (ctl->fused && ctl->batch_n >= 2) {
         ctl->n_fused += 1;
         if (ctl->commit_n == ctl->batch_n) ctl->cur ^= 1u;
@@ -3812,7 +3940,7 @@
     const dim3 grid(tile_grid(v.n_tiles, v.n_cus, occ[slot_mode(v.endbit)], kLutThreads)), block(kLutThreads);
     const int hot_launched = w.hot;
 #define MBPE_FUSED_ARGS v.tok, v.tok_other, v.sums, v.side, v.n_tiles, v.chg, b.bs, b.hdr_adj, b.LR, v.ctl, v.left_edge, \
-                        v.right_edge, b.hdr_m, v.run_in, hot_launched, b.pair_cells
+                        v.right_edge, b.hdr_m, v.run_in, hot_launched, b.pair_cells, v.slow_list
 #ifdef MBPE_DIAG
     const int diag = getenv("MBPE_FUSED_DIAG") ? atoi(getenv("MBPE_FUSED_DIAG")) : 0;
 #define MBPE_FUSED_DIAG_CASE(D)                                                                                            \
@@ -3829,6 +3957,19 @@
 #undef MBPE_FUSED_DIAG_CASE
 #endif
     MBPE_BY_MODE(v.endbit, MBPE_BY_INST(w, hipLaunchKernelGGL((k_fused_batch<M, HOT, TT>), grid, block, 0, v.stream, MBPE_FUSED_ARGS)));
+    if (v.slow_list) {
+        const dim3 slow_grid(v.n_cus > 0 ? v.n_cus : 256);
+        MBPE_BY_MODE(v.endbit, {
+            MBPE_BY_INST(w, hipLaunchKernelGGL((k_fused_batch<M, HOT, TT, 0, true>), grid, block, 0, v.stream, MBPE_FUSED_ARGS));
+            if (w.known && w.tt && !w.hot)
+                hipLaunchKernelGGL((k_fused_batch<M, false, false, 0, true>), grid, block, 0, v.stream, MBPE_FUSED_ARGS);
+            if (w.known && w.tt && w.hot)
+                hipLaunchKernelGGL((k_fused_batch<M, true, false, 0, true>), grid, block, 0, v.stream, MBPE_FUSED_ARGS);
+            hipLaunchKernelGGL((k_fused_slow<M>), slow_grid, block, 0, v.stream, v.tok, v.tok_other, v.sums, v.side, v.n_tiles,
+                               v.chg, b.bs, b.hdr_adj, b.LR, v.ctl, v.left_edge, v.right_edge, b.hdr_m, v.run_in,
+                               b.pair_cells, v.slow_list);
+        });
+    }
 #undef MBPE_FUSED_ARGS
 }
 
@@ -3922,7 +4063,7 @@
 }
 
 void launch_seq_finish(const StreamView &v, const BatchView &b, uint32_t *fused_flag) {
-    hipLaunchKernelGGL(k_seq_finish, dim3(1), dim3(64), 0, v.stream, v.ctl, fused_flag, b.bs);
+    hipLaunchKernelGGL(k_seq_finish, dim3(1), dim3(64), 0, v.stream, v.ctl, fused_flag, b.bs, v.n_tiles);
 }
 
 void launch_tile_scan(const StreamView &v, unsigned long long *offsets) {
diff --git a/minbpe-cc_amd/csrc/mbpe_dev.h b/minbpe-cc_amd/csrc/mbpe_dev.h
--- a/minbpe-cc_amd/csrc/mbpe_dev.h
+++ b/minbpe-cc_amd/csrc/mbpe_dev.h
@@ -99,7 +99,10 @@
     uint32_t cell_hits;
     uint32_t cells_min;
     uint32_t adj_pitch;
-
+    uint32_t slow_on;
+    uint32_t slow_n;
+    uint32_t slow_off;
+    unsigned long long n_slow_tiles;
 };
 
 #ifndef MBPE_BATCH_MAX
@@ -172,6 +175,7 @@
     uint32_t n_tiles;
     uint32_t *chg;
     uint32_t *tile_list;
+    uint32_t *slow_list;
     uint32_t *run_in;
     unsigned long long *run_part;
     DevCtl *ctl;
diff --git a/minbpe-cc_amd/csrc/train.cpp b/minbpe-cc_amd/csrc/train.cpp
--- a/minbpe-cc_amd/csrc/train.cpp
+++ b/minbpe-cc_amd/csrc/train.cpp
@@ -113,6 +113,7 @@
     TileSum *side = nullptr;
     uint32_t *chg = nullptr;
     uint32_t *tile_list = nullptr;
+    uint32_t *slow_list = nullptr;
     SelList *sel = nullptr;
     uint32_t *run_in = nullptr;
     int seq_slot = -1;
@@ -174,6 +175,7 @@
     uint32_t *h_seq = nullptr;
     uint32_t *d_seq_info = nullptr;
     int64_t opt_pair_cells = -1;
+    int64_t opt_slow_tiles = -1;
     int64_t opt_lockstep = -1;
     hipEvent_t ev_sel = nullptr;
     std::vector<hipEvent_t> kev;
@@ -277,7 +279,7 @@
 
 void free_training(mbpe_ctx *c) {
     tfree(c, c->tok[0]); tfree(c, c->tok[1]);
-    tfree(c, c->sums); tfree(c, c->side); tfree(c, c->chg); tfree(c, c->tile_list);
+    tfree(c, c->sums); tfree(c, c->side); tfree(c, c->chg); tfree(c, c->tile_list); tfree(c, c->slow_list);
     tfree(c, c->offsets);
     tfree(c, c->tab.hslot); tfree(c, c->tab.ekey); tfree(c, c->tab.ecnt); tfree(c, c->tab.cells);
     tfree(c, c->tab.bmax); tfree(c, c->tab.smax);
@@ -419,7 +421,7 @@
     v.stream = c->stream;
     v.tok = c->tok[first], v.tok_other = c->tok[1 - first];
     v.sums = c->sums, v.side = c->side, v.n_tiles = c->n_tiles;
-    v.chg = c->chg, v.tile_list = c->tile_list;
+    v.chg = c->chg, v.tile_list = c->tile_list, v.slow_list = c->slow_list;
     v.run_in = c->run_in, v.run_part = c->offsets + c->n_tiles;
     v.ctl = c->ctl;
     v.left_edge = multi ? c->d_left : nullptr, v.right_edge = multi ? c->d_right : nullptr;
@@ -538,6 +540,7 @@
     else if (n == "byte_table") c->opt_byte_table = value != 0;
     else if (n == "lockstep") c->opt_lockstep = value < 0 ? -1 : value != 0;
     else if (n == "pair_cells") c->opt_pair_cells = value < 0 ? -1 : value != 0;
+    else if (n == "slow_tiles") c->opt_slow_tiles = value < 0 ? -1 : value != 0;
     else if (n == "wide_from") c->opt_wide_from = value < 0 ? -1 : value;
     else if (n == "first_wide") c->opt_first_wide = value != 0;
     else if (n == "pc_repeat") c->opt_pc_repeat = std::min<int64_t>(std::max<int64_t>(1, value), 1000);
@@ -757,6 +760,11 @@
     return c->h_ctl.n_entries > (1u << 20);
 }
 
+static inline bool use_lockstep(const mbpe_ctx *c);
+static bool use_slow_tiles(const mbpe_ctx *c) {
+    return c->opt_slow_tiles > 0 || (c->opt_slow_tiles < 0 && !use_lockstep(c));
+}
+
 static int begin_local(mbpe_ctx *c, uint32_t vocab_size) {
     free_training(c);
     c->vocab_size = vocab_size;
@@ -786,6 +794,7 @@
     HIPCHK(tmalloc(c, &c->side, (size_t)c->n_tiles * sizeof(TileSum)));
     HIPCHK(tmalloc(c, &c->chg, ((size_t)c->n_tiles / 32 + 2) * 4));
     HIPCHK(tmalloc(c, &c->tile_list, ((size_t)c->n_tiles + 64) * 4));
+    if (use_slow_tiles(c)) HIPCHK(tmalloc(c, &c->slow_list, ((size_t)c->n_tiles + 64) * 4));
     HIPCHK(hipMemsetAsync(c->chg, 0, ((size_t)c->n_tiles / 32 + 2) * 4, c->stream));
     HIPCHK(tmalloc(c, &c->offsets, ((size_t)c->n_tiles + tile_scan_scratch(c->n_tiles)) * 8));
     const size_t xb_words = (size_t)c->hdr_words + c->hdrb_words + lr_words(vocab_size, c->max_batch_eff) + 8;
@@ -828,6 +837,7 @@
         init.adj_pitch = c->adj_pitch;
         init.cells_on = c->pair_cells ? 1u : 0u;
         init.cells_min = c->opt_pair_cells > 0 ? 2u : kCellsMinBatch;
+        init.slow_on = !c->slow_list ? 0u : c->opt_slow_tiles > 0 ? 2u : 1u;
         c->h_ctl = init;
         HIPCHK(hipMemcpyAsync(c->ctl, &c->h_ctl, sizeof(DevCtl), hipMemcpyHostToDevice, c->stream));
     }
@@ -1493,6 +1503,7 @@
     c->h_wbest.clear();
     c->wide_active = true;
     tfree(c, c->tok[0]); tfree(c, c->tok[1]); tfree(c, c->sums); tfree(c, c->side); tfree(c, c->chg); tfree(c, c->tile_list);
+    tfree(c, c->slow_list);
     tfree(c, c->offsets); tfree(c, c->run_in); tfree(c, c->xb); tfree(c, c->pair_cells);
     tfree(c, c->tab.hslot); tfree(c, c->tab.ekey); tfree(c, c->tab.ecnt); tfree(c, c->tab.bmax); tfree(c, c->tab.smax);
     tfree(c, c->first_state);
@@ -1728,6 +1739,8 @@
     for (int i = 0; i < 8; ++i) c->stats.size_hist[i] = c->begun ? c->h_ctl.size_hist[i] : 0;
     c->stats.n_skipped = c->begun ? c->h_ctl.n_skipped : 0;
     c->stats.n_skip_cut = c->begun ? c->h_ctl.n_skip_cut : 0;
+    c->stats.n_slow_tiles = c->begun ? c->h_ctl.n_slow_tiles : 0;
+    c->stats.slow_tiles_off = c->begun ? c->h_ctl.slow_off : 0;
     if (c->begun && c->wide_active) {
         c->stats.n_slots = c->h_wctl.n;
         c->stats.n_live = c->h_wctl.n;
diff --git a/minbpe-cc_amd/python/mbpe/__init__.py b/minbpe-cc_amd/python/mbpe/__init__.py
--- a/minbpe-cc_amd/python/mbpe/__init__.py
+++ b/minbpe-cc_amd/python/mbpe/__init__.py
@@ -49,7 +49,8 @@
         ("n_sel_retry", ctypes.c_uint32), ("adapt_limit", ctypes.c_uint32), ("n_sel_blocks", ctypes.c_uint64), ("size_hist", ctypes.c_uint32 * 8),
         ("n_skipped", ctypes.c_uint32), ("n_skip_cut", ctypes.c_uint32),
         ("exchange_words", ctypes.c_uint64), ("exchanges", ctypes.c_uint32), ("pad_", ctypes.c_uint32),
-        ("fused_live_tokens", ctypes.c_uint64), ("ms_pair_count_kernel", ctypes.c_float), ("pad2_", ctypes.c_uint32),
+        ("fused_live_tokens", ctypes.c_uint64), ("ms_pair_count_kernel", ctypes.c_float), ("slow_tiles_off", ctypes.c_uint32),
+        ("n_slow_tiles", ctypes.c_uint64),
     ]
 
     def as_dict(self):
```

Result: slower. 78650 merges/s (-2.1%).
